# openzklib/openzl

Measured on AMD Instinct MI355X. Metric: MSM points/sec (BLS12-381 G1), higher is better.
Workload: dtype u32; 1 GPU; bls12_381_g1_msm_2^24_per_gpu; points_per_gpu=16777216, curve=BLS12-381 G1, scalars=uniform < r (255 bit), window_bits=20, windows=13, precomputed_table=none (the fixed-key table mode is reported separately as msm_fixed_key), parallelism=single

## Files before the change

### openzl_amd/csrc/zl_msm_accumulate.h

```cpp
#pragma once
#include <type_traits>
#include "zl_ctx.h"
#include "zl_quad.h"
#include "zl_fq2pair.h"
#include "zl_msm_common.h"

__device__ __forceinline__ uint32_t zl_upper_bound(const uint32_t* __restrict__ a, uint32_t n, uint32_t key) {
    uint32_t lo = 0, hi = n;
    while (lo < hi) {
        uint32_t mid = (lo + hi) >> 1;
        if (a[mid] <= key) lo = mid + 1; else hi = mid;
    }
    return lo;
}

#ifndef ZL_ACC_WAVES
#define ZL_ACC_WAVES 2
#endif
#ifndef ZL_ACC_BLOCK
#define ZL_ACC_BLOCK 64
#endif
template <class G, bool QUAD = false>
__device__ __forceinline__ void zl_accumulate_chunk(uint32_t t, int sub, uint32_t E, const uint32_t* __restrict__ entries, const uint32_t* __restrict__ offsets, uint32_t NB,
                                                    const Affine<typename HotField<typename G::F>::type>* __restrict__ bases,
                                                    XYZZ<typename HotField<typename G::F>::type>* __restrict__ bucket_sums,
                                                    XYZZ<typename HotField<typename G::F>::type>* __restrict__ partials, uint32_t ZL_CHUNK,
                                                    const Affine<typename HotField<typename G::F>::type>* __restrict__ phib, uint32_t n_real, uint32_t idx_mask = 0x7fffffffu) {
    using F = typename HotField<typename G::F>::type;
    const uint64_t start64 = (uint64_t)t * ZL_CHUNK;
    if (start64 >= E) return;
    const uint32_t start = (uint32_t)start64;
    const uint32_t end = (uint32_t)min((uint64_t)E, start64 + ZL_CHUNK);
    uint32_t b = zl_upper_bound(offsets, NB + 1, start) - 1;
    uint32_t b_start = offsets[b], b_end = offsets[b + 1];
    XYZZ<F> acc = XYZZ<F>::inf();
    for (uint32_t e = start; e < end; e++) {
        while (e == b_end) {
            if (b_end > b_start) {
                if (!QUAD || sub == 0) {
                    if (b_start >= start) bucket_sums[b] = acc;
                    else partials[(size_t)2 * t] = acc;
                }
                acc = XYZZ<F>::inf();
            }
            b++;
            b_start = b_end;
            b_end = offsets[b + 1];
        }
        const uint32_t ent = entries[e];
        const uint32_t idx = ent & idx_mask;
        const Affine<F> P = (G::GLV && idx >= n_real ? phib : bases)[idx];
        if (!P.is_inf()) {
            if constexpr (QUAD) zl::add_mixed_quad(acc, P.x, P.y, (ent >> 31) != 0, sub);
            else zl::add_mixed(acc, P.x, P.y, (ent >> 31) != 0);
        }
    }
    const bool complete = (b_start >= start) && (b_end <= end);
    if (QUAD && sub != 0) return;
    if (complete) bucket_sums[b] = acc;
    else partials[(size_t)2 * t + (b_start <= start ? 0 : 1)] = acc;
}
template <class G>
__global__ void __launch_bounds__(ZL_ACC_BLOCK, ZL_ACC_WAVES * 64 / ZL_ACC_BLOCK > 0 ? ZL_ACC_WAVES * 64 / ZL_ACC_BLOCK : 1) k_msm_accumulate(const uint32_t* __restrict__ entries, const uint32_t* __restrict__ offsets, uint32_t NB,
                                                        const Affine<typename G::F>* __restrict__ bases_,
                                                        XYZZ<typename G::F>* __restrict__ bucket_sums_,
                                                        XYZZ<typename G::F>* __restrict__ partials_, uint32_t ZL_CHUNK,
                                                        const Affine<typename G::F>* __restrict__ phib_, uint32_t n_real) {
    using F = typename HotField<typename G::F>::type;
    static_assert(sizeof(F) == sizeof(typename G::F), "hot flavour must share the layout");
    zl_accumulate_chunk<G>(blockIdx.x * blockDim.x + threadIdx.x, 0, offsets[NB], entries, offsets, NB, reinterpret_cast<const Affine<F>*>(bases_),
                           reinterpret_cast<XYZZ<F>*>(bucket_sums_), reinterpret_cast<XYZZ<F>*>(partials_), ZL_CHUNK,
                           reinterpret_cast<const Affine<F>*>(phib_) - n_real, n_real);
}
#ifdef ZL_MEASURE
template <class G>
__global__ void __launch_bounds__(ZL_ACC_BLOCK, ZL_ACC_WAVES * 64 / ZL_ACC_BLOCK > 0 ? ZL_ACC_WAVES * 64 / ZL_ACC_BLOCK : 1) k_msm_accumulate_clk(const uint32_t* __restrict__ entries, const uint32_t* __restrict__ offsets, uint32_t NB,
                                                        const Affine<typename G::F>* __restrict__ bases_,
                                                        XYZZ<typename G::F>* __restrict__ bucket_sums_,
                                                        XYZZ<typename G::F>* __restrict__ partials_, uint32_t ZL_CHUNK,
                                                        const Affine<typename G::F>* __restrict__ phib_, uint32_t n_real, unsigned long long* __restrict__ clk, uint32_t idx_mask) {
    if constexpr (G::COORDS == 1) {
        using F = typename HotField<typename G::F>::type;
        const unsigned long long c0 = __builtin_readcyclecounter(), w0 = __builtin_amdgcn_s_memrealtime();
        zl_accumulate_chunk<G>(blockIdx.x * blockDim.x + threadIdx.x, 0, offsets[NB], entries, offsets, NB, reinterpret_cast<const Affine<F>*>(bases_),
                               reinterpret_cast<XYZZ<F>*>(bucket_sums_), reinterpret_cast<XYZZ<F>*>(partials_), ZL_CHUNK,
                               reinterpret_cast<const Affine<F>*>(phib_) - n_real, n_real, idx_mask);
        const unsigned long long c1 = __builtin_readcyclecounter(), w1 = __builtin_amdgcn_s_memrealtime();
        if (threadIdx.x == 0) {
            unsigned long long* o = clk + (size_t)4 * blockIdx.x;
            o[0] = c0; o[1] = c1; o[2] = w0; o[3] = w1;
        }
    }
}
#endif
template <class G>
__global__ void __launch_bounds__(ZL_ACC_BLOCK, ZL_ACC_WAVES * 64 / ZL_ACC_BLOCK > 0 ? ZL_ACC_WAVES * 64 / ZL_ACC_BLOCK : 1) k_msm_accumulate_quad(const uint32_t* __restrict__ entries, const uint32_t* __restrict__ offsets, uint32_t NB,
                                                        const Affine<typename G::F>* __restrict__ bases_,
                                                        XYZZ<typename G::F>* __restrict__ bucket_sums_,
                                                        XYZZ<typename G::F>* __restrict__ partials_, uint32_t ZL_CHUNK,
                                                        const Affine<typename G::F>* __restrict__ phib_, uint32_t n_real) {
    using F = typename HotField<typename G::F>::type;
    const uint32_t gt = blockIdx.x * blockDim.x + threadIdx.x;
    zl_accumulate_chunk<G, true>(gt >> 2, (int)(gt & 3u), offsets[NB], entries, offsets, NB, reinterpret_cast<const Affine<F>*>(bases_),
                                 reinterpret_cast<XYZZ<F>*>(bucket_sums_), reinterpret_cast<XYZZ<F>*>(partials_), ZL_CHUNK,
                                 reinterpret_cast<const Affine<F>*>(phib_) - n_real, n_real);
}
#ifndef ZL_ACC_PAIR_WAVES
#define ZL_ACC_PAIR_WAVES 2
#endif
template <class G, bool QUAD = false>
__global__ void __launch_bounds__(64, ZL_ACC_PAIR_WAVES) k_msm_accumulate_pair(const uint32_t* __restrict__ entries, const uint32_t* __restrict__ offsets, uint32_t NB,
                                                        const Affine<typename G::F>* __restrict__ bases_,
                                                        XYZZ<typename G::F>* __restrict__ bucket_sums,
                                                        XYZZ<typename G::F>* __restrict__ partials, uint32_t ZL_CHUNK,
                                                        const Affine<typename G::F>* __restrict__ phib_, uint32_t n_real) {
    using B = typename PairBase<typename G::F>::type;
    static_assert(!std::is_void<B>::value, "lane-pair kernels: Fq2 groups on 28-bit limbs only");
    using H = Fp2H<B>;
    const int half = zl::pair_half(), sub = (int)(threadIdx.x & 3u);
    const uint32_t t = QUAD ? ZL_OCTET_ITEM() : ZL_PAIR_ITEM();
    const uint32_t E = offsets[NB];
    const Affine<typename G::F>* __restrict__ phib = phib_ - n_real;
    const uint64_t start64 = (uint64_t)t * ZL_CHUNK;
    if (start64 >= E) return;
    const uint32_t start = (uint32_t)start64;
    const uint32_t end = (uint32_t)min((uint64_t)E, start64 + ZL_CHUNK);
    uint32_t b = zl_upper_bound(offsets, NB + 1, start) - 1;
    uint32_t b_start = offsets[b], b_end = offsets[b + 1];
    XYZZ<H> acc = XYZZ<H>::inf();
    for (uint32_t e = start; e < end; e++) {
        while (e == b_end) {
            if (b_end > b_start) {
                if (b_start >= start) pair_store(&bucket_sums[b], half, acc);
                else pair_store(&partials[(size_t)2 * t], half, acc);
                acc = XYZZ<H>::inf();
            }
            b++;
            b_start = b_end;
            b_end = offsets[b + 1];
        }
        const uint32_t ent = entries[e];
        const uint32_t idx = ent & 0x7fffffffu;
        const Affine<H> P = pair_load(&(G::GLV && idx >= n_real ? phib : bases_)[idx], half);
        if (!P.is_inf()) {
            if constexpr (QUAD) zl::add_mixed_quad(acc, P.x, P.y, (ent >> 31) != 0, sub);
            else zl::add_mixed(acc, P.x, P.y, (ent >> 31) != 0);
        }
    }
    const bool complete = (b_start >= start) && (b_end <= end);
    if (complete) pair_store(&bucket_sums[b], half, acc);
    else pair_store(&partials[(size_t)2 * t + (b_start <= start ? 0 : 1)], half, acc);
}
#ifdef ZL_MEASURE
#define ZL_MSM_ACCUMULATE_CLK_KERNEL(X, G) X template __global__ void k_msm_accumulate_clk<G>(const uint32_t*, const uint32_t*, uint32_t, const Affine<typename G::F>*, XYZZ<typename G::F>*, XYZZ<typename G::F>*, uint32_t, const Affine<typename G::F>*, uint32_t, unsigned long long*, uint32_t);
#else
#define ZL_MSM_ACCUMULATE_CLK_KERNEL(X, G)
#endif
#define ZL_MSM_ACCUMULATE_KERNELS_G1(X, G) \
    ZL_MSM_ACCUMULATE_CLK_KERNEL(X, G) \
    X template __global__ void k_msm_accumulate<G>(const uint32_t*, const uint32_t*, uint32_t, const Affine<typename G::F>*, XYZZ<typename G::F>*, XYZZ<typename G::F>*, uint32_t, const Affine<typename G::F>*, uint32_t); \
    X template __global__ void k_msm_accumulate_quad<G>(const uint32_t*, const uint32_t*, uint32_t, const Affine<typename G::F>*, XYZZ<typename G::F>*, XYZZ<typename G::F>*, uint32_t, const Affine<typename G::F>*, uint32_t);
#define ZL_MSM_ACCUMULATE_KERNELS_G2(X, G) \
    X template __global__ void k_msm_accumulate_pair<G, true>(const uint32_t*, const uint32_t*, uint32_t, const Affine<typename G::F>*, XYZZ<typename G::F>*, XYZZ<typename G::F>*, uint32_t, const Affine<typename G::F>*, uint32_t); \
    X template __global__ void k_msm_accumulate_pair<G, false>(const uint32_t*, const uint32_t*, uint32_t, const Affine<typename G::F>*, XYZZ<typename G::F>*, XYZZ<typename G::F>*, uint32_t, const Affine<typename G::F>*, uint32_t);
```

### openzl_amd/csrc/zl_msm_job.h

```cpp
#pragma once
#include <chrono>
#include <stdlib.h>
#include <string.h>
#include <stdio.h>
#include <algorithm>
#include <vector>
#include "zl_ctx.h"
#include "zl_pool.h"
#include "zl_msm_sort.h"
#include "zl_msm_endo.h"
#include "zl_msm_accumulate.h"
#include "zl_msm_reduce.h"

#ifndef ZL_GLS_HOLE_LO_LOG
#define ZL_GLS_HOLE_LO_LOG 11
#define ZL_GLS_HOLE_HI_LOG 17
#define ZL_GLS_END_LOG 19
#endif
static_assert(ZL_GLS_HOLE_LO_LOG >= 0 && ZL_GLS_HOLE_LO_LOG <= ZL_GLS_HOLE_HI_LOG && ZL_GLS_HOLE_HI_LOG <= ZL_GLS_END_LOG && ZL_GLS_END_LOG <= 32, "split below 2^END outside [2^LO, 2^HI)");

static int zl_pick_window(size_t n, int sc_bits, bool wide16 = false ) {
    const double per_bucket = (double)zl_tune("ZL_TUNE_BUCKET_COST_X10", sc_bits > 200 ? 45 : 52) / 10.0;
    double best = 1e300;
    int best_c = 2;
    for (int c = 2; c <= 20; c++) {
        int W = (sc_bits + 1 + c - 1) / c;
        if (c > 16 && (((uint64_t)W << (c - 1)) >> 15) > 255) continue;
        const bool lds_sort = c < 16 || (c == 16 && !wide16);
        double cost = (double)n * W * (lds_sort ? 1.10 : 1.0) + per_bucket * W * (double)(1u << (c - 1));
        if (cost < best) { best = cost; best_c = c; }
    }
    return best_c;
}

static int zl_pick_window_half(size_t n_points) {
    if (n_points < 2) return 0;
    int lg = 63 - __builtin_clzll((unsigned long long)n_points);
    if ((double)n_points >= 1.4142 * (double)((size_t)1 << lg)) lg++;
    static const signed char best[9] = {9, 0, 11, 12, 0, 0, 0, 16, 0};
    return lg >= 11 && lg <= 19 ? best[lg - 11] : 0;
}
static int zl_pick_window_quarter(size_t n_points) {
    if (n_points < 2) return 0;
    int lg = 63 - __builtin_clzll((unsigned long long)n_points);
    if ((double)n_points >= 1.4142 * (double)((size_t)1 << lg)) lg++;
    static const signed char best[9] = {9, 0, 11, 12, 13, 13, 13, 13, 14};
    return lg >= 10 && lg <= 18 ? best[lg - 10] : 0;
}

static int zl_pick_window_precomp(size_t n, int sc_bits) {
    if (n < (size_t)700000) return 16;
    if (n < ((size_t)1 << 21)) return 20;
    double best = 1e300;
    int best_c = 16;
    for (int c = 20; c <= 23; c++) {
        int W = (sc_bits + 1 + c - 1) / c;
        double cost = (double)n * W + 6.0 * (double)(1u << (c - 1));
        if (cost < best) { best = cost; best_c = c; }
    }
    return best_c;
}

struct MsmSortLayout {
    size_t a_bytes = 0, b_bytes = 0;
    uint32_t nslices = 0, per_slice = 0;
    size_t hi8 = 0, part_lo = 0, part_idx = 0, pcounts = 0, idx2 = 0, counts2 = 0;
    uint32_t P = 0, pscan_blocks = 0, fsl = 0, P2 = 0, p2scan_blocks = 0;
    size_t slice_counts = 0;
    size_t vs = 0;
};
template <class G>
struct MsmJob {
    using F = typename G::F;
    using X = XYZZ<F>;
    bool pre = false;
    int c = 0, W = 0;
    int spread_t = -1;
    bool wide = false;
    bool glv = false;
    bool phi_cached = false;
    bool phi_owner = false;
    int sc_bits = 0, endo_k = 1;
    zl_slot phi_slot = ZL_SLOT_PHI_ONE_KEY;
    MsmSortLayout lay;
    unsigned char *d_sort_a = nullptr, *d_sort_b = nullptr;
    size_t n_real = 0;
    uint32_t* d_vs = nullptr;
    const Affine<F>* d_phi = nullptr;
    uint32_t H = 0, SETS = 0, NB = 0, ZL_CHUNK = 0, nchunks = 0, scan_blocks = 0, max_big = 0, max_giant = 0, Gn = 0, big_span = ZL_BIG_SPAN;
    uint32_t red_g0 = 0, red_lg0 = 0, red_blocks = 0, red_levels = 0;
    uint32_t roots_per_set = 0;
    uint64_t maxE = 0;
    size_t n = 0, first = 0;
    const zl_bases* bsp = nullptr;
    uint32_t *d_counts = nullptr, *d_offsets = nullptr, *d_cursor = nullptr, *d_entries = nullptr, *d_block_sums = nullptr, *d_big_list = nullptr,
             *d_big_count = nullptr, *d_ones_count = nullptr, *d_giant_count = nullptr, *d_giant_list = nullptr, *d_ones_list = nullptr,
             *d_bigsg_items = nullptr, *d_bad_scalar = nullptr;
    unsigned long long* d_bigsg_head = nullptr;
    X *d_buckets = nullptr, *d_partials = nullptr, *d_segs = nullptr, *d_stage1 = nullptr, *d_sets = nullptr, *d_ones_parts = nullptr, *d_giant_tmp = nullptr;
    const Affine<F>* d_bases = nullptr;
    const uint8_t* d_inf = nullptr;
    const uint32_t* sc = nullptr;
    X* hw = nullptr;
    uint32_t* hE = nullptr;
    std::vector<X> hw_own;
    void set_host_buffer(X* buf) {
        hw = buf;
        hE = reinterpret_cast<uint32_t*>(buf + (size_t)SETS * roots_per_set + 1);
    }

    int plan(zl_ctx* ctx, const zl_bases& bs, size_t first_, const void* d_scalars, size_t n_, zl_slot phi_slot_) {
        static const bool no_glv = getenv("ZL_NO_GLV") != nullptr;
        bool try_glv = false;
        static const size_t glv_max = (size_t)1 << zl_tune("ZL_TUNE_GLV_MAX_LOG", 19);
        if constexpr (G::GLV) try_glv = bs.precomp_c == 0 && !no_glv && n_ >= 1 && n_ <= glv_max && (uint64_t)n_ * G::ENDO_K < (1ull << 31);
        if constexpr (G::GLV && G::ENDO_K == 2) {
            if constexpr (G::GLVP::LATTICE) {
                if (n_ >= ((size_t)1 << 13) && n_ < ((size_t)1 << 17)) try_glv = false;
            }
        }
        if constexpr (G::GLV && G::ENDO_K == 4) {
            if constexpr (G::GLVP::LATTICE) {
                if (((uint64_t)n_ >= (1ull << ZL_GLS_HOLE_LO_LOG) && (uint64_t)n_ < (1ull << ZL_GLS_HOLE_HI_LOG)) || (uint64_t)n_ >= (1ull << ZL_GLS_END_LOG)) try_glv = false;
            }
        }
        int rc = plan_as(ctx, bs, first_, d_scalars, n_, try_glv);
        if (!rc && glv && c <= 3) rc = plan_as(ctx, bs, first_, d_scalars, n_, false);
        if (!rc && glv && !wide && c > 16) rc = plan_as(ctx, bs, first_, d_scalars, n_, false);
        phi_slot = phi_slot_;
        phi_owner = glv;
        return rc;
    }
    int plan_as(zl_ctx* ctx, const zl_bases& bs, size_t first_, const void* d_scalars, size_t n_, bool glv_) {
        glv = glv_;
        n_real = n_;
        endo_k = glv ? (int)G::ENDO_K : 1;
        n = (size_t)endo_k * n_;
        sc_bits = !glv ? (int)G::SC_BITS : MsmJobPartBits<G>::value;
        first = first_;
        bsp = &bs;
        pre = bs.precomp_c > 0;
        c = pre ? bs.precomp_c : (ctx->msm_c > 0 ? ctx->msm_c : zl_pick_window(n, sc_bits, glv && G::ENDO_K != 2));
        if (!pre && ctx->msm_c <= 0 && glv) {
            int h = 0;
            if constexpr (G::ENDO_K == 2) {
                if (!G::GLVP::LATTICE) h = zl_pick_window_half(n_);
            } else {
                h = zl_pick_window_quarter(n_);
            }
            if (h) c = h;
        }
        if (c < 2) c = 2;
        if (c > 24) c = 24;
        W = (sc_bits + 1 + c - 1) / c;
        H = 1u << (c - 1);
        SETS = pre ? 1u : (uint32_t)W;
        const uint64_t NB64 = (uint64_t)SETS * H;
        maxE = (uint64_t)n * W;
        if (n >= (1ull << 31) || maxE >= (1ull << 32) || NB64 >= (1ull << 31)) return ZL_EINVAL;
        if (pre && (uint64_t)W * bs.n >= (1ull << 31)) return ZL_EINVAL;
        NB = (uint32_t)NB64;
        Gn = NB >> 15;
        if (pre && (c < 16 || Gn < 1 || Gn > 255)) return ZL_EINVAL;
        wide = pre || ((c > 16 || (glv && c == 16 && G::ENDO_K != 2)) && Gn >= 1 && Gn <= 255);
        ZL_CHUNK = (maxE >> 7) >= (1u << 20) ? 128u : (uint32_t)ZL_CHUNK_MAX;
        while (ZL_CHUNK > 8 && maxE / ZL_CHUNK < (1u << 18)) ZL_CHUNK >>= 1;
        uint32_t dense = glv && G::ENDO_K == 2 ? 2u : 1u;
        if constexpr (G::GLV && G::ENDO_K == 4) {
            if constexpr (G::GLVP::LATTICE) {
                static_assert(G::GLVP::PEAK_PCT <= 400, "the top window's busiest buckets are more than 4x the average: a factor of 2 no longer keeps them below 8 chunks");
                if (glv && G::GLVP::PEAK_PCT > 200) dense = 2u;
            }
        }
        while (ZL_CHUNK < (uint32_t)ZL_CHUNK_MAX && dense * (maxE / std::max<uint64_t>(1, (uint64_t)SETS * H)) > (uint64_t)4 * ZL_CHUNK) ZL_CHUNK <<= 1;
        ZL_CHUNK = (uint32_t)std::max(8, zl_tune("ZL_TUNE_CHUNK", (int)ZL_CHUNK));
        nchunks = (uint32_t)((maxE + ZL_CHUNK - 1) / ZL_CHUNK);
        {
            uint32_t g0 = NB >= (1u << 20) ? 8u : (NB >= (1u << 17) ? 4u : 2u);
            g0 = (uint32_t)std::max(2, zl_tune("ZL_TUNE_SEG", (int)g0));
            while (g0 & (g0 - 1)) g0 &= g0 - 1;
            if (g0 > H) g0 = H;
            spread_t = -1;
            if ((wide || c <= 16) && !pre) {
                const int top_bits = sc_bits + 1 - (W - 1) * c;
                if (top_bits - 1 < c - 1) {
                    spread_t = top_bits - 1;
                    if (spread_t > 0 && (1u << spread_t) < g0) g0 = 1u << spread_t;
                }
            }
            red_g0 = g0;
            red_lg0 = 31 - __builtin_clz(g0);
            red_blocks = H / g0;
            red_levels = 31 - __builtin_clz(red_blocks);
            roots_per_set = red_levels + 2;
        }
        scan_blocks = (NB + SCAN_BLOCK * SCAN_ITEMS - 1) / (SCAN_BLOCK * SCAN_ITEMS);
        big_span = nchunks <= (1u << 17) ? (uint32_t)ZL_BIG_SPAN_SMALL : (uint32_t)ZL_BIG_SPAN;
        max_big = (uint32_t)(maxE / ((uint64_t)ZL_CHUNK * big_span)) + 1;
        max_giant = (uint32_t)(maxE / ((uint64_t)ZL_CHUNK * ZL_GIANT_SPAN)) + 1;
        lay = MsmSortLayout{};
        auto up256 = [](size_t b) { return (b + 255) / 256 * 256; };
        const uint32_t max_slices = (uint32_t)((n + 4095) / 4096);
        if (wide) {
            lay.nslices = std::min<uint32_t>(64, max_slices);
            lay.P = Gn * W * lay.nslices;
            lay.pscan_blocks = (lay.P + SCAN_BLOCK * SCAN_ITEMS - 1) / (SCAN_BLOCK * SCAN_ITEMS);
            const size_t b_lo = up256((size_t)n * W * 2), b_hi = up256((size_t)n * W), b_idx = up256((size_t)n * W * 4);
            lay.hi8 = b_lo;
            lay.part_lo = lay.hi8 + b_hi;
            lay.part_idx = lay.part_lo + b_lo;
            lay.pcounts = lay.part_idx + b_idx;
            lay.a_bytes = lay.pcounts + up256((size_t)(2 * lay.P + lay.pscan_blocks + 8) * 4) + 256;
            lay.fsl = 16;
            while (lay.fsl * Gn < 2048 && lay.fsl < 128) lay.fsl *= 2;
            lay.P2 = Gn * 128 * lay.fsl;
            lay.p2scan_blocks = (lay.P2 + SCAN_BLOCK * SCAN_ITEMS - 1) / (SCAN_BLOCK * SCAN_ITEMS);
            lay.idx2 = b_lo;
            lay.counts2 = lay.idx2 + b_idx;
            lay.b_bytes = lay.counts2 + up256((size_t)(2 * (size_t)lay.P2 + lay.p2scan_blocks + 8) * 4) + 256;
        } else if (c <= 16) {
            lay.nslices = std::max<uint32_t>(1, std::min<uint32_t>((256 + W - 1) / W, max_slices));
            lay.slice_counts = up256((size_t)n * W * 2);
            lay.a_bytes = (size_t)n * W * 2 + (size_t)lay.nslices * NB * 4 + 256;
        }
        if (lay.nslices) lay.per_slice = (uint32_t)((n + lay.nslices - 1) / lay.nslices);
        if (glv) {
            lay.vs = up256(lay.a_bytes);
            lay.a_bytes = lay.vs + up256((size_t)n * 32);
        }
        d_bases = pre ? reinterpret_cast<const Affine<F>*>(bs.d_table) : reinterpret_cast<const Affine<F>*>(bs.d_pts) + first;
        d_inf = bs.d_inf ? reinterpret_cast<const uint8_t*>(bs.d_inf) + first : nullptr;
        sc = reinterpret_cast<const uint32_t*>(d_scalars);
        hw_own.assign((size_t)SETS * roots_per_set + 2, X::inf());
        set_host_buffer(hw_own.data());
        return ZL_OK;
    }
    int alloc(zl_ctx* ctx, int set, bool own_sort = false) {
        void* p;
        int rc;
        const zl_msm_set_slots& slots = ZL_MSM_SET[set];
        d_sort_a = d_sort_b = nullptr;
        if (lay.a_bytes) {
            if ((rc = zl_scratch_get(ctx, own_sort ? slots.sort_a : ZL_SLOT_SORT_A, lay.a_bytes, &p))) return rc;
            d_sort_a = (unsigned char*)p;
        }
        if (lay.b_bytes) {
            if ((rc = zl_scratch_get(ctx, own_sort ? slots.sort_b : ZL_SLOT_SORT_B, lay.b_bytes, &p))) return rc;
            d_sort_b = (unsigned char*)p;
        }
        const size_t max_bigsg = (size_t)(maxE / 1024) + 2;
        size_t small_words = (size_t)3 * (NB + 1) + 1 + scan_blocks + 1 + max_big + max_giant + 16 + n + 2 * max_bigsg;
        if ((rc = zl_scratch_get(ctx, slots.data[0], small_words * 4, &p))) return rc;
        d_counts = (uint32_t*)p;
        d_offsets = d_counts + (NB + 1);
        d_cursor = d_offsets + (NB + 2);
        d_block_sums = d_cursor + (NB + 1);
        d_big_list = d_block_sums + scan_blocks + 1;
        d_big_count = d_big_list + max_big;
        d_ones_count = d_big_count + 1;
        d_giant_count = d_big_count + 2;
        d_bad_scalar = d_big_count + 3;
        d_giant_list = d_big_count + 16;
        d_ones_list = d_giant_list + max_giant;
        d_bigsg_items = d_ones_list + n;
        d_bigsg_head = reinterpret_cast<unsigned long long*>((reinterpret_cast<uintptr_t>(d_big_count + 4) + 7) & ~(uintptr_t)7);
        if ((rc = zl_scratch_get(ctx, slots.data[1], maxE * 4, &p))) return rc;
        d_entries = (uint32_t*)p;
        if ((rc = zl_scratch_get(ctx, slots.data[2], (size_t)NB * sizeof(X), &p))) return rc;
        d_buckets = (X*)p;
        if ((rc = zl_scratch_get(ctx, slots.data[3], (size_t)2 * nchunks * sizeof(X), &p))) return rc;
        d_partials = (X*)p;
        const size_t leaf_elems = (size_t)2 * SETS * red_blocks, lvl1_elems = (size_t)3 * SETS * (red_blocks / 2 + 1);
        const size_t root_elems = (size_t)SETS * roots_per_set;
        if ((rc = zl_scratch_get(ctx, slots.tail, (leaf_elems + lvl1_elems + root_elems + 2 + ZL_ONES_BLOCKS + (size_t)max_giant * ZL_GIANT_PARTS) * sizeof(X), &p))) return rc;
        d_segs = (X*)p;
        d_stage1 = d_segs + leaf_elems;
        d_sets = d_stage1 + lvl1_elems;
        d_ones_parts = d_sets + root_elems + 2;
        d_giant_tmp = d_ones_parts + ZL_ONES_BLOCKS;
        if (glv) {
            const size_t endo_bytes = (size_t)(endo_k - 1) * n_real * sizeof(Affine<F>);
            const zl_bases& bs = *bsp;
            std::lock_guard<std::mutex> cache_lk(zl_bases_cache_mutex());
            if (!bs.d_endo && endo_bytes <= ((size_t)zl_tune("ZL_TUNE_ENDO_CACHE_MB", 512) << 20)) {
                void* q = nullptr;
                if (hipMalloc(&q, endo_bytes) == hipSuccess) {
                    if constexpr (G::GLV && G::ENDO_K == 2)
                        hipLaunchKernelGGL((k_glv_phi<G>), dim3((uint32_t)((n_real + 127) / 128)), dim3(128), 0, ctx->stream, d_bases, (uint32_t)n_real, reinterpret_cast<Affine<F>*>(q));
                    else if constexpr (G::GLV && G::ENDO_K == 4)
                        hipLaunchKernelGGL((k_gls_psi<G>), dim3((uint32_t)((n_real + 63) / 64)), dim3(64), 0, ctx->stream, d_bases, (uint32_t)n_real, reinterpret_cast<Affine<F>*>(q));
                    if (hipGetLastError() != hipSuccess || hipStreamSynchronize(ctx->stream) != hipSuccess) { (void)hipFree(q); return ZL_EHIP; }
                    bs.d_endo = q;
                    bs.endo_first = first;
                    bs.endo_n = n_real;
                    bs.endo_k = endo_k;
                } else {
                    (void)hipGetLastError();
                }
            }
            if (bs.d_endo && bs.endo_first == first && bs.endo_n == n_real && bs.endo_k == endo_k) {
                d_phi = reinterpret_cast<const Affine<F>*>(bs.d_endo);
                phi_owner = false;
                phi_cached = true;
            }
        }
        if (glv && phi_owner) {
            if ((rc = zl_scratch_get(ctx, phi_slot, (size_t)(endo_k - 1) * n_real * sizeof(Affine<F>), &p))) return rc;
            d_phi = reinterpret_cast<const Affine<F>*>(p);
        }
        return ZL_OK;
    }
    int sort(zl_ctx* ctx, hipStream_t st) {
        if (!wide && c > 16) ZL_HIP(ctx, hipMemsetAsync(d_counts, 0, (size_t)(NB + 1) * 4, st));
        hipLaunchKernelGGL(k_msm_zero_words, dim3(1), dim3(64), 0, st, d_big_count, 8u);
        const uint32_t nblk = (uint32_t)((n + 255) / 256);
        const uint32_t* sc_eff = sc;
        const uint8_t* inf_eff = d_inf;
        uint32_t* bad_eff = d_bad_scalar;
        if (glv) {
            d_vs = reinterpret_cast<uint32_t*>(d_sort_a + lay.vs);
            if constexpr (G::GLV && G::ENDO_K == 2) {
                if constexpr (G::GLVP::LATTICE)
                    hipLaunchKernelGGL((k_glv_split_lattice<typename G::GLVP>), dim3((uint32_t)((n_real + 255) / 256)), dim3(256), 0, st, sc, (uint32_t)n_real, d_inf, d_vs, (int)G::SC_BITS, d_bad_scalar);
                else
                    hipLaunchKernelGGL((k_glv_split<typename G::GLVP>), dim3((uint32_t)((n_real + 255) / 256)), dim3(256), 0, st, sc, (uint32_t)n_real, d_inf, d_vs, (int)G::SC_BITS, d_bad_scalar);
                if (phi_owner)
                    hipLaunchKernelGGL((k_glv_phi<G>), dim3((uint32_t)((n_real + 127) / 128)), dim3(128), 0, st, d_bases, (uint32_t)n_real, const_cast<Affine<F>*>(d_phi));
            } else if constexpr (G::GLV && G::ENDO_K == 4) {
                if constexpr (G::GLVP::LATTICE)
                    hipLaunchKernelGGL((k_gls_split_lattice<typename G::GLVP>), dim3((uint32_t)((n_real + 255) / 256)), dim3(256), 0, st, sc, (uint32_t)n_real, d_inf, d_vs, (int)G::SC_BITS, d_bad_scalar);
                else
                    hipLaunchKernelGGL((k_gls_split<typename G::GLVP>), dim3((uint32_t)((n_real + 255) / 256)), dim3(256), 0, st, sc, (uint32_t)n_real, d_inf, d_vs, (int)G::SC_BITS, d_bad_scalar);
                if (phi_owner)
                    hipLaunchKernelGGL((k_gls_psi<G>), dim3((uint32_t)((n_real + 63) / 64)), dim3(64), 0, st, d_bases, (uint32_t)n_real, const_cast<Affine<F>*>(d_phi));
            }
            sc_eff = d_vs;
            inf_eff = nullptr;
            bad_eff = nullptr;
        }
        const int glv_i = glv ? 1 : 0;
        (void)hipFuncSetAttribute(reinterpret_cast<const void*>(&k_msm_hist_lds), hipFuncAttributeMaxDynamicSharedMemorySize, 128 * 1024);
        (void)hipFuncSetAttribute(reinterpret_cast<const void*>(&k_msm_scatter_range), hipFuncAttributeMaxDynamicSharedMemorySize, 128 * 1024);
        if (wide) sort_wide(st, sc_eff, inf_eff, bad_eff, nblk, glv_i);
        else if (c <= 16) sort_lds(st, sc_eff, inf_eff, bad_eff, nblk, glv_i);
        else sort_atomics(st, nblk);
        ZL_HIP(ctx, hipGetLastError());
        return ZL_OK;
    }
    void sort_wide(hipStream_t st, const uint32_t* sc_eff, const uint8_t* inf_eff, uint32_t* bad_eff, uint32_t nblk, int glv_i) {
        const zl_bases& bs = *bsp;
        const uint32_t nslices = lay.nslices, per_slice = lay.per_slice, P = lay.P, pscan_blocks = lay.pscan_blocks;
        uint16_t* d_lo16 = (uint16_t*)d_sort_a;
        uint8_t* d_hi8 = (uint8_t*)(d_sort_a + lay.hi8);
        uint16_t* d_part_lo = (uint16_t*)(d_sort_a + lay.part_lo);
        uint32_t* d_part_idx = (uint32_t*)(d_sort_a + lay.part_idx);
        uint32_t* d_pcounts = (uint32_t*)(d_sort_a + lay.pcounts);
        uint32_t* d_poff = d_pcounts + P;
        uint32_t* d_pblock = d_poff + P + 1;
        hipLaunchKernelGGL(k_msm_recode_wide, dim3(nblk), dim3(256), 0, st, sc_eff, (uint32_t)n, c, W, pre ? 0u : (H >> 15), spread_t, glv_i, d_lo16, d_hi8, d_ones_list, d_ones_count, inf_eff, sc_bits, bad_eff);
        hipLaunchKernelGGL(k_msm_part_hist, dim3(nslices, W), dim3(256), 0, st, d_hi8, (uint32_t)n, (uint32_t)W, Gn, per_slice, nslices, d_pcounts);
        hipLaunchKernelGGL(k_scan_block_sums, dim3(pscan_blocks), dim3(SCAN_BLOCK), 0, st, d_pcounts, P, d_pblock);
        hipLaunchKernelGGL(k_scan_top, dim3(1), dim3(1024), 0, st, d_pblock, pscan_blocks, d_poff + P, (const uint32_t*)nullptr);
        hipLaunchKernelGGL(k_scan_apply, dim3(pscan_blocks), dim3(SCAN_BLOCK), 0, st, d_pcounts, P, d_pblock, d_poff, d_pcounts);
        hipLaunchKernelGGL(k_msm_part_scatter_st, dim3(nslices, W), dim3(256), 0, st, d_lo16, d_hi8, (uint32_t)n, (uint32_t)W, Gn, per_slice, nslices, d_poff,
                           pre ? (uint32_t)bs.n : 0u, pre ? (uint32_t)first : 0u, d_part_lo, d_part_idx);
        const uint32_t gstride = (uint32_t)W * nslices;
        const uint32_t SG = Gn * 128;
        const uint32_t fsl = lay.fsl, P2 = lay.P2, p2scan_blocks = lay.p2scan_blocks;
        uint16_t* d_lo2 = (uint16_t*)d_sort_b;
        uint32_t* d_idx2 = (uint32_t*)(d_sort_b + lay.idx2);
        uint32_t* d_c2 = (uint32_t*)(d_sort_b + lay.counts2);
        uint32_t* d_off2 = d_c2 + P2;
        uint32_t* d_blk2 = d_off2 + P2 + 1;
        hipLaunchKernelGGL(k_msm_sub_hist, dim3(fsl, Gn), dim3(256), 0, st, d_part_lo, d_poff, Gn, gstride, d_poff + P, fsl, d_c2);
        hipLaunchKernelGGL(k_scan_block_sums, dim3(p2scan_blocks), dim3(SCAN_BLOCK), 0, st, d_c2, P2, d_blk2);
        hipLaunchKernelGGL(k_scan_top, dim3(1), dim3(1024), 0, st, d_blk2, p2scan_blocks, d_off2 + P2, (const uint32_t*)nullptr);
        hipLaunchKernelGGL(k_scan_apply, dim3(p2scan_blocks), dim3(SCAN_BLOCK), 0, st, d_c2, P2, d_blk2, d_off2, d_c2);
        hipLaunchKernelGGL(k_msm_sub_scatter_st, dim3(fsl, Gn), dim3(256), 0, st, d_part_lo, d_part_idx, d_poff, Gn, gstride, d_poff + P, fsl, d_off2, d_lo2,
                           d_idx2);
        hipLaunchKernelGGL(k_msm_fine_hist, dim3(SG), dim3(256), 0, st, d_lo2, d_off2, SG, fsl, d_off2 + P2, d_counts);
        hipLaunchKernelGGL(k_scan_block_sums, dim3(scan_blocks), dim3(SCAN_BLOCK), 0, st, d_counts, NB, d_block_sums);
        hipLaunchKernelGGL(k_scan_top, dim3(1), dim3(1024), 0, st, d_block_sums, scan_blocks, d_offsets + NB, (const uint32_t*)d_bad_scalar);
        hipLaunchKernelGGL(k_scan_apply, dim3(scan_blocks), dim3(SCAN_BLOCK), 0, st, d_counts, NB, d_block_sums, d_offsets, d_cursor);
        uint32_t cap = (uint32_t)std::min<uint64_t>(36 * 1024, std::max<uint64_t>(4096, (maxE / SG) * 22 / 10));
        cap = (uint32_t)std::max(1024, zl_tune("ZL_TUNE_FS_CAP", (int)cap));
        (void)hipFuncSetAttribute(reinterpret_cast<const void*>(&k_msm_fine_sort), hipFuncAttributeMaxDynamicSharedMemorySize, 160 * 1024);
        hipLaunchKernelGGL(k_msm_fine_sort, dim3(SG), dim3(zl_tune("ZL_TUNE_FS", 1024)), (size_t)(256 + cap) * 4, st, d_lo2, d_idx2, d_off2, SG, fsl, d_off2 + P2, d_offsets, cap,
                           d_entries, d_bigsg_head, d_bigsg_items);
        (void)hipFuncSetAttribute(reinterpret_cast<const void*>(&k_msm_fine_sort_big), hipFuncAttributeMaxDynamicSharedMemorySize, ZL_BT * 4);
        hipLaunchKernelGGL(k_msm_fine_sort_big, dim3(512), dim3(1024), (size_t)ZL_BT * 4, st, d_lo2, d_idx2, d_off2, SG, fsl, d_off2 + P2, d_bigsg_head,
                           d_bigsg_items, d_cursor, d_entries);
    }
    void sort_lds(hipStream_t st, const uint32_t* sc_eff, const uint8_t* inf_eff, uint32_t* bad_eff, uint32_t nblk, int glv_i) {
        const uint32_t nslices = lay.nslices, per_slice = lay.per_slice;
        uint16_t* d_digits = (uint16_t*)d_sort_a;
        uint32_t* d_slice_counts = (uint32_t*)(d_sort_a + lay.slice_counts);
        hipLaunchKernelGGL(k_msm_recode, dim3(nblk), dim3(256), 0, st, sc_eff, (uint32_t)n, c, W, spread_t, glv_i, d_digits, d_ones_list, d_ones_count, inf_eff, sc_bits, bad_eff);
        hipLaunchKernelGGL(k_msm_hist_lds, dim3(nslices, W), dim3(1024), (size_t)H * 4, st, d_digits, (uint32_t)n, H, per_slice, NB, d_slice_counts);
        if (NB <= 14336 && nslices <= 64) {
            hipLaunchKernelGGL(k_msm_prefix_small, dim3(1), dim3(1024), ((size_t)NB + NB / 16 + 16) * 4, st, d_slice_counts, NB, nslices, d_offsets, d_cursor, (const uint32_t*)d_bad_scalar);
        } else {
        hipLaunchKernelGGL(k_msm_slice_prefix, dim3((NB + 255) / 256), dim3(256), 0, st, d_slice_counts, NB, nslices, d_counts);
        hipLaunchKernelGGL(k_scan_block_sums, dim3(scan_blocks), dim3(SCAN_BLOCK), 0, st, d_counts, NB, d_block_sums);
        hipLaunchKernelGGL(k_scan_top, dim3(1), dim3(1024), 0, st, d_block_sums, scan_blocks, d_offsets + NB, (const uint32_t*)d_bad_scalar);
        hipLaunchKernelGGL(k_scan_apply, dim3(scan_blocks), dim3(SCAN_BLOCK), 0, st, d_counts, NB, d_block_sums, d_offsets, d_cursor);
        }
        uint32_t ranges = 1;
        while (ranges * W < 256 && (H / (ranges * 2)) >= 64) ranges *= 2;
        ranges = (uint32_t)std::max(1, zl_tune("ZL_TUNE_RANGES", (int)ranges));
        const uint32_t RB = (H + ranges - 1) / ranges;
        const uint32_t parts = 1;
        hipLaunchKernelGGL(k_msm_scatter_range, dim3(8 * ((W + 7) / 8), ranges, parts), dim3(1024), (size_t)RB * 4, st, d_digits, (uint32_t)n, H, RB, d_offsets, d_entries,
                           (const uint32_t*)d_slice_counts, NB, nslices, per_slice, parts, (uint32_t)W);
    }
    void sort_atomics(hipStream_t st, uint32_t nblk) {
        hipLaunchKernelGGL((k_msm_digits<0>), dim3(nblk), dim3(256), 0, st, sc, (uint32_t)n, c, W, d_counts, (uint32_t*)nullptr, d_ones_list, d_ones_count, d_inf, (int)G::SC_BITS, d_bad_scalar);
        hipLaunchKernelGGL(k_scan_block_sums, dim3(scan_blocks), dim3(SCAN_BLOCK), 0, st, d_counts, NB, d_block_sums);
        hipLaunchKernelGGL(k_scan_top, dim3(1), dim3(1024), 0, st, d_block_sums, scan_blocks, d_offsets + NB, (const uint32_t*)d_bad_scalar);
        hipLaunchKernelGGL(k_scan_apply, dim3(scan_blocks), dim3(SCAN_BLOCK), 0, st, d_counts, NB, d_block_sums, d_offsets, d_cursor);
        hipLaunchKernelGGL((k_msm_digits<1>), dim3(nblk), dim3(256), 0, st, sc, (uint32_t)n, c, W, d_cursor, d_entries, d_ones_list, d_ones_count, d_inf, (int)G::SC_BITS, d_bad_scalar);
    }
    static constexpr bool pair_ok() { return G::COORDS == 2 && !std::is_void<typename PairBase<F>::type>::value; }
    int accumulate(zl_ctx* ctx, hipStream_t st) {
        static_assert(G::COORDS == 1 || pair_ok(), "every Fq2 group runs on 28-bit limbs: its MSM kernels are the lane-pair ones");
        const bool quad = nchunks <= (uint64_t)zl_tune("ZL_TUNE_QUAD_ACC_CHUNKS", 24576);
        if constexpr (pair_ok()) {
            if (quad)
                hipLaunchKernelGGL((k_msm_accumulate_pair<G, true>), dim3((nchunks + 7) / 8), dim3(64), 0, st, d_entries, d_offsets, NB, d_bases, d_buckets, d_partials, ZL_CHUNK,
                                   glv ? d_phi : d_bases, glv ? (uint32_t)n_real : 0xFFFFFFFFu);
            else
                hipLaunchKernelGGL((k_msm_accumulate_pair<G, false>), dim3((nchunks + 31) / 32), dim3(64), 0, st, d_entries, d_offsets, NB, d_bases, d_buckets, d_partials, ZL_CHUNK,
                                   glv ? d_phi : d_bases, glv ? (uint32_t)n_real : 0xFFFFFFFFu);
        } else {
            if (quad)
                hipLaunchKernelGGL((k_msm_accumulate_quad<G>), dim3((4 * nchunks + ZL_ACC_BLOCK - 1) / ZL_ACC_BLOCK), dim3(ZL_ACC_BLOCK), 0, st, d_entries, d_offsets, NB, d_bases, d_buckets, d_partials, ZL_CHUNK,
                                   glv ? d_phi : d_bases, glv ? (uint32_t)n_real : 0xFFFFFFFFu);
#ifdef ZL_MEASURE
            else if (ctx->acc_clk && (size_t)((nchunks + ZL_ACC_BLOCK - 1) / ZL_ACC_BLOCK) * 32 <= ctx->acc_clk_cap) {
                ctx->acc_clk_waves = (nchunks + ZL_ACC_BLOCK - 1) / ZL_ACC_BLOCK;
                hipLaunchKernelGGL((k_msm_accumulate_clk<G>), dim3((nchunks + ZL_ACC_BLOCK - 1) / ZL_ACC_BLOCK), dim3(ZL_ACC_BLOCK), 0, st, d_entries, d_offsets, NB, d_bases, d_buckets, d_partials, ZL_CHUNK,
                                   glv ? d_phi : d_bases, glv ? (uint32_t)n_real : 0xFFFFFFFFu, (unsigned long long*)ctx->acc_clk,
                                   zl_tune("ZL_TUNE_ACC_CLK_IDX_BITS", 31) >= 31 ? 0x7fffffffu : ((1u << zl_tune("ZL_TUNE_ACC_CLK_IDX_BITS", 31)) - 1u));
            }
#endif
            else
                hipLaunchKernelGGL((k_msm_accumulate<G>), dim3((nchunks + ZL_ACC_BLOCK - 1) / ZL_ACC_BLOCK), dim3(ZL_ACC_BLOCK), 0, st, d_entries, d_offsets, NB, d_bases, d_buckets, d_partials, ZL_CHUNK,
                                   glv ? d_phi : d_bases, glv ? (uint32_t)n_real : 0xFFFFFFFFu);
        }
        ZL_HIP(ctx, hipGetLastError());
        return ZL_OK;
    }
    int tail(zl_ctx* ctx, hipStream_t st) {
        const uint32_t quad_max = (uint32_t)zl_tune("ZL_TUNE_QUAD_LANES", 65536);
        const bool by_cuts = NB > quad_max && nchunks > 1;
        if (by_cuts) hipLaunchKernelGGL((k_msm_fill_empty<G>), dim3((NB + 255) / 256), dim3(256), 0, st, d_offsets, NB, d_buckets);
        if constexpr (pair_ok()) {
            if (by_cuts)
                hipLaunchKernelGGL((k_msm_merge_cuts_pair<G>), dim3((nchunks + 31) / 32), dim3(64), 0, st, d_offsets, NB, d_buckets, d_partials, d_big_list, d_big_count, d_giant_list, d_giant_count, ZL_CHUNK, big_span, nchunks);
            else if (NB > quad_max)
                hipLaunchKernelGGL((k_msm_merge_pair<G, false>), dim3((NB + 31) / 32), dim3(64), 0, st, d_offsets, NB, d_buckets, d_partials, d_big_list, d_big_count, d_giant_list, d_giant_count, ZL_CHUNK, big_span);
            else
                hipLaunchKernelGGL((k_msm_merge_pair<G, true>), dim3((NB + 7) / 8), dim3(64), 0, st, d_offsets, NB, d_buckets, d_partials, d_big_list, d_big_count, d_giant_list, d_giant_count, ZL_CHUNK, big_span);
        } else {
            if (by_cuts)
                hipLaunchKernelGGL((k_msm_merge_cuts<G>), dim3((nchunks + 63) / 64), dim3(64), 0, st, d_offsets, NB, d_buckets, d_partials, d_big_list, d_big_count, d_giant_list, d_giant_count, ZL_CHUNK, big_span, nchunks);
            else if (NB > quad_max)
                hipLaunchKernelGGL((k_msm_merge<G>), dim3((NB + 63) / 64), dim3(64), 0, st, d_offsets, NB, d_buckets, d_partials, d_big_list, d_big_count, d_giant_list, d_giant_count, ZL_CHUNK, big_span);
            else
                hipLaunchKernelGGL((k_msm_merge<G, true>), dim3((4 * NB + 63) / 64), dim3(64), 0, st, d_offsets, NB, d_buckets, d_partials, d_big_list, d_big_count, d_giant_list, d_giant_count, ZL_CHUNK, big_span);
        }
        const bool may_big = nchunks > big_span, may_giant = nchunks > (uint32_t)ZL_GIANT_SPAN;
        if constexpr (pair_ok()) {
            if (may_big) hipLaunchKernelGGL((k_msm_merge_big_pair<G>), dim3(std::min<uint32_t>(max_big, 1024)), dim3(2 * TreeLanes<G>::N), TreeLanes<G>::N * sizeof(X), st, d_offsets, d_buckets,
                               d_partials, d_big_list, d_big_count, ZL_CHUNK);
            if (may_giant) hipLaunchKernelGGL((k_msm_merge_giant_pair<G>), dim3(std::min<uint32_t>(max_giant, 16) * ZL_GIANT_PARTS), dim3(2 * TreeLanes<G>::N), TreeLanes<G>::N * sizeof(X), st,
                               d_offsets, d_giant_tmp, d_partials, d_giant_list, d_giant_count, ZL_CHUNK);
            if (may_giant) hipLaunchKernelGGL((k_msm_merge_giant2_pair<G>), dim3(std::min<uint32_t>(max_giant, 64)), dim3(2 * ZL_GIANT_PARTS), 0, st, d_buckets, d_giant_tmp, d_giant_list, d_giant_count);
        } else {
            if (may_big) hipLaunchKernelGGL((k_msm_merge_big<G>), dim3(std::min<uint32_t>(max_big, 1024)), dim3(TreeLanes<G>::N), TreeLanes<G>::N * sizeof(X), st, d_offsets, d_buckets,
                           d_partials, d_big_list, d_big_count, ZL_CHUNK);
            if (may_giant) hipLaunchKernelGGL((k_msm_merge_giant<G>), dim3(std::min<uint32_t>(max_giant, 16) * ZL_GIANT_PARTS), dim3(TreeLanes<G>::N), TreeLanes<G>::N * sizeof(X), st,
                           d_offsets, d_giant_tmp, d_partials, d_giant_list, d_giant_count, ZL_CHUNK);
            if (may_giant) hipLaunchKernelGGL((k_msm_merge_giant2<G>), dim3((max_giant + 63) / 64), dim3(64), 0, st, d_buckets, d_giant_tmp, d_giant_list, d_giant_count);
        }
        hipLaunchKernelGGL((k_msm_ones<G>), dim3(ZL_ONES_BLOCKS), dim3(TreeLanes<G>::N), TreeLanes<G>::N * sizeof(X), st, d_ones_list, d_ones_count,
                           pre ? d_bases + first : d_bases, d_ones_parts, glv ? d_phi : d_bases, glv ? (uint32_t)n_real : 0xFFFFFFFFu,
                           d_sets + (size_t)SETS * roots_per_set, d_big_count + 6, (const uint32_t*)(d_offsets + NB));
        {
            const uint32_t fset = spread_t >= 0 ? (uint32_t)(W - 1) : 0xFFFFFFFFu, flog = (uint32_t)std::max(spread_t, 0);
            const uint32_t leaves = SETS * red_blocks;
            X* cur = red_levels == 0 ? d_sets : d_segs;
            if constexpr (pair_ok()) {
                if (leaves > quad_max)
                    hipLaunchKernelGGL((k_msm_reduce_level0_pair<G, false>), dim3((leaves + 31) / 32), dim3(64), 0, st, d_buckets, H, red_g0, red_blocks, leaves, fset, flog, cur);
                else
                    hipLaunchKernelGGL((k_msm_reduce_level0_pair<G, true>), dim3((leaves + 7) / 8), dim3(64), 0, st, d_buckets, H, red_g0, red_blocks, leaves, fset, flog, cur);
            } else {
                if (leaves > quad_max)
                    hipLaunchKernelGGL((k_msm_reduce_level0<G>), dim3((leaves + 63) / 64), dim3(64), 0, st, d_buckets, H, red_g0, red_blocks, leaves, fset, flog, cur);
                else
                    hipLaunchKernelGGL((k_msm_reduce_level0<G, true>), dim3((4 * leaves + 63) / 64), dim3(64), 0, st, d_buckets, H, red_g0, red_blocks, leaves, fset, flog, cur);
            }
            for (uint32_t lv = 1; lv <= red_levels; lv++) {
                const uint32_t nodes = red_blocks >> lv, lanes = SETS * nodes * (lv + 2);
                X* nxt = lv == red_levels ? d_sets : ((lv & 1) ? d_stage1 : d_segs);
                if constexpr (pair_ok()) {
                    if (lanes > quad_max)
                        hipLaunchKernelGGL((k_msm_reduce_tree_pair<G, false>), dim3((lanes + 31) / 32), dim3(64), 0, st, cur, nxt, lv, nodes, lanes);
                    else
                        hipLaunchKernelGGL((k_msm_reduce_tree_pair<G, true>), dim3((lanes + 7) / 8), dim3(64), 0, st, cur, nxt, lv, nodes, lanes);
                } else {
                    if (lanes > quad_max)
                        hipLaunchKernelGGL((k_msm_reduce_tree<G>), dim3((lanes + 63) / 64), dim3(64), 0, st, cur, nxt, lv, nodes, lanes);
                    else
                        hipLaunchKernelGGL((k_msm_reduce_tree<G, true>), dim3((4 * lanes + 63) / 64), dim3(64), 0, st, cur, nxt, lv, nodes, lanes);
                }
                cur = nxt;
            }
        }
        ZL_HIP(ctx, hipGetLastError());
        ZL_HIP(ctx, hipMemcpyAsync(hw, d_sets, sizeof(X) * ((size_t)SETS * roots_per_set + 1) + 8, hipMemcpyDeviceToHost, st));
        return ZL_OK;
    }
    X window_value(int w) const {
        const X* root = hw + (size_t)w * roots_per_set;
        X v = X::inf();
        const int top = (int)red_lg0 + (int)red_levels - 1;
        for (int off = std::max(top, 0); off >= 0; off--) {
            if (off != std::max(top, 0)) zl::dbl_inplace(v);
            const int bsel = off - (int)red_lg0;
            if (bsel >= 0 && bsel < (int)red_levels) {
                const bool skipped = spread_t >= 0 && w == (int)SETS - 1 && off >= spread_t && !pre;
                if (!skipped) zl::add_full(v, root[2 + bsel]);
            }
            if (off == 0) zl::add_full(v, root[1]);
        }
        return v;
    }
    X finish(bool parallel = true, double* values_us = nullptr) const {
        std::vector<X> V(SETS);
        const auto t0 = std::chrono::steady_clock::now();
        if (parallel && SETS >= 4) zl_pool_get().parallel_for(SETS, [&](size_t w) { V[w] = window_value((int)w); });
        else for (uint32_t w = 0; w < SETS; w++) V[w] = window_value((int)w);
        if (values_us) *values_us = (double)std::chrono::duration_cast<std::chrono::nanoseconds>(std::chrono::steady_clock::now() - t0).count() / 1e3;
        X total = V[SETS - 1];
        for (int w = (int)SETS - 2; w >= 0; w--) {
            zl::dbl_n(total, c);
            zl::add_full(total, V[w]);
        }
        zl::add_full(total, hw[(size_t)SETS * roots_per_set]);
        return total;
    }
};
```

### openzl_amd/csrc/zl_msm_reduce.h

```cpp
#pragma once
#include "zl_ctx.h"
#include <type_traits>
#include "zl_quad.h"
#include "zl_fq2pair.h"
#include "zl_msm_common.h"

template <class G, bool QUAD = false>
__global__ void __launch_bounds__(64, (QUAD && sizeof(XYZZ<typename G::F>) <= 256) ? 3 : 1) k_msm_merge(const uint32_t* __restrict__ offsets, uint32_t NB, XYZZ<typename G::F>* __restrict__ bucket_sums,
                                                   const XYZZ<typename G::F>* __restrict__ partials, uint32_t* __restrict__ big_list,
                                                   uint32_t* __restrict__ big_count, uint32_t* __restrict__ giant_list, uint32_t* __restrict__ giant_count,
                                                   uint32_t ZL_CHUNK, uint32_t big_span) {
    ZL_SIDE_PRIO();
    using F = typename G::F;
    const uint32_t gt = blockIdx.x * blockDim.x + threadIdx.x;
    const uint32_t b = QUAD ? gt >> 2 : gt;
    const int sub = QUAD ? (int)(gt & 3u) : 0;
    if (b >= NB) return;
    const uint32_t s = offsets[b], e = offsets[b + 1];
    if (s == e) { if (sub == 0) bucket_sums[b] = XYZZ<F>::inf(); return; }
    const uint32_t t0 = s / ZL_CHUNK, t1 = (e - 1) / ZL_CHUNK;
    if (t0 == t1) return;
    if (t1 - t0 + 1 > ZL_GIANT_SPAN) { if (sub == 0) giant_list[atomicAdd(giant_count, 1u)] = b; return; }
    if (t1 - t0 + 1 > big_span) { if (sub == 0) big_list[atomicAdd(big_count, 1u)] = b; return; }
    XYZZ<F> acc = XYZZ<F>::inf();
    for (uint32_t t = t0; t <= t1; t++) {
        const XYZZ<F> p = partials[(size_t)2 * t + (s <= t * ZL_CHUNK ? 0 : 1)];
        if constexpr (QUAD) zl::add_full_quad(acc, p, sub);
        else zl::add_full(acc, p);
    }
    if (sub == 0) bucket_sums[b] = acc;
}
__device__ __forceinline__ uint32_t zl_bucket_of_entry(const uint32_t* __restrict__ offsets, uint32_t NB, uint32_t p) {
    uint32_t lo = 0, hi = NB + 1;
    while (lo < hi) {
        const uint32_t mid = (lo + hi) >> 1;
        if (offsets[mid] <= p) lo = mid + 1; else hi = mid;
    }
    return lo - 1;
}
template <class G>
__global__ void __launch_bounds__(256) k_msm_fill_empty(const uint32_t* __restrict__ offsets, uint32_t NB, XYZZ<typename G::F>* __restrict__ bucket_sums) {
    ZL_SIDE_PRIO();
    const uint32_t b = blockIdx.x * blockDim.x + threadIdx.x;
    if (b >= NB || offsets[b] != offsets[b + 1]) return;
    bucket_sums[b] = XYZZ<typename G::F>::inf();
}
template <class G>
__global__ void __launch_bounds__(64, sizeof(XYZZ<typename G::F>) <= 256 ? 3 : 1) k_msm_merge_cuts(const uint32_t* __restrict__ offsets, uint32_t NB, XYZZ<typename G::F>* __restrict__ bucket_sums,
                                                   const XYZZ<typename G::F>* __restrict__ partials, uint32_t* __restrict__ big_list,
                                                   uint32_t* __restrict__ big_count, uint32_t* __restrict__ giant_list, uint32_t* __restrict__ giant_count,
                                                   uint32_t ZL_CHUNK, uint32_t big_span, uint32_t nchunks) {
    ZL_SIDE_PRIO();
    using F = typename G::F;
    const uint32_t t = blockIdx.x * blockDim.x + threadIdx.x + 1;
    if (t >= nchunks) return;
    const uint64_t p64 = (uint64_t)t * ZL_CHUNK;
    if (p64 >= offsets[NB]) return;
    const uint32_t p = (uint32_t)p64;
    const uint32_t b = zl_bucket_of_entry(offsets, NB, p);
    const uint32_t s = offsets[b], e = offsets[b + 1];
    if (s == p || s / ZL_CHUNK != t - 1) return;
    const uint32_t t0 = t - 1, t1 = (e - 1) / ZL_CHUNK;
    if (t1 - t0 + 1 > ZL_GIANT_SPAN) { giant_list[atomicAdd(giant_count, 1u)] = b; return; }
    if (t1 - t0 + 1 > big_span) { big_list[atomicAdd(big_count, 1u)] = b; return; }
    XYZZ<F> acc = XYZZ<F>::inf();
    for (uint32_t tt = t0; tt <= t1; tt++) {
        const XYZZ<F> q = partials[(size_t)2 * tt + (s <= tt * ZL_CHUNK ? 0 : 1)];
        zl::add_full(acc, q);
    }
    bucket_sums[b] = acc;
}
template <class G>
struct TreeLanes { static constexpr int N = sizeof(XYZZ<typename G::F>) > 256 ? 128 : 256; };
template <class G>
__device__ __forceinline__ void zl_block_tree(XYZZ<typename G::F>* sh, XYZZ<typename G::F>& acc) {
    using F = typename G::F;
    sh[threadIdx.x] = acc;
    __syncthreads();
    for (int off = TreeLanes<G>::N / 2; off > 0; off >>= 1) {
        if ((int)threadIdx.x < off) {
            XYZZ<F> a = sh[threadIdx.x];
            const XYZZ<F> o = sh[threadIdx.x + off];
            zl::add_full(a, o);
            sh[threadIdx.x] = a;
        }
        __syncthreads();
    }
    acc = sh[0];
    __syncthreads();
}
template <class G>
__global__ void __launch_bounds__(TreeLanes<G>::N) k_msm_merge_big(const uint32_t* __restrict__ offsets, XYZZ<typename G::F>* __restrict__ bucket_sums,
                                                        const XYZZ<typename G::F>* __restrict__ partials, const uint32_t* __restrict__ big_list,
                                                        const uint32_t* __restrict__ big_count, uint32_t ZL_CHUNK) {
    ZL_SIDE_PRIO();
    using F = typename G::F;
    extern __shared__ __attribute__((aligned(16))) unsigned char smem[];
    XYZZ<F>* sh = reinterpret_cast<XYZZ<F>*>(smem);
    for (uint32_t item = blockIdx.x; item < *big_count; item += gridDim.x) {
        const uint32_t b = big_list[item];
        const uint32_t s = offsets[b], e = offsets[b + 1];
        const uint32_t t0 = s / ZL_CHUNK, t1 = (e - 1) / ZL_CHUNK;
        XYZZ<F> acc = XYZZ<F>::inf();
        for (uint32_t t = t0 + threadIdx.x; t <= t1; t += blockDim.x) {
            const XYZZ<F> p = partials[(size_t)2 * t + (s <= t * ZL_CHUNK ? 0 : 1)];
            zl::add_full(acc, p);
        }
        zl_block_tree<G>(sh, acc);
        if (threadIdx.x == 0) bucket_sums[b] = acc;
    }
}
template <class G>
__global__ void __launch_bounds__(TreeLanes<G>::N) k_msm_merge_giant(const uint32_t* __restrict__ offsets, XYZZ<typename G::F>* __restrict__ giant_tmp,
                                                          const XYZZ<typename G::F>* __restrict__ partials, const uint32_t* __restrict__ giant_list,
                                                          const uint32_t* __restrict__ giant_count, uint32_t ZL_CHUNK) {
    ZL_SIDE_PRIO();
    using F = typename G::F;
    extern __shared__ __attribute__((aligned(16))) unsigned char smem[];
    XYZZ<F>* sh = reinterpret_cast<XYZZ<F>*>(smem);
    const uint32_t part = blockIdx.x % ZL_GIANT_PARTS;
    for (uint32_t item = blockIdx.x / ZL_GIANT_PARTS; item < *giant_count; item += gridDim.x / ZL_GIANT_PARTS) {
        const uint32_t b = giant_list[item];
        const uint32_t s = offsets[b], e = offsets[b + 1];
        const uint32_t t0 = s / ZL_CHUNK, t1 = (e - 1) / ZL_CHUNK;
        const uint32_t per = (t1 - t0 + ZL_GIANT_PARTS) / ZL_GIANT_PARTS;
        const uint32_t lo = t0 + part * per, hi = min(t1 + 1, lo + per);
        XYZZ<F> acc = XYZZ<F>::inf();
        for (uint32_t t = lo + threadIdx.x; t < hi; t += blockDim.x) {
            const XYZZ<F> p = partials[(size_t)2 * t + (s <= t * ZL_CHUNK ? 0 : 1)];
            zl::add_full(acc, p);
        }
        zl_block_tree<G>(sh, acc);
        if (threadIdx.x == 0) giant_tmp[(size_t)item * ZL_GIANT_PARTS + part] = acc;
    }
}
template <class G>
__global__ void __launch_bounds__(64) k_msm_merge_giant2(XYZZ<typename G::F>* __restrict__ bucket_sums, const XYZZ<typename G::F>* __restrict__ giant_tmp,
                                                          const uint32_t* __restrict__ giant_list, const uint32_t* __restrict__ giant_count) {
    ZL_SIDE_PRIO();
    using F = typename G::F;
    const uint32_t item = blockIdx.x * blockDim.x + threadIdx.x;
    if (item >= *giant_count) return;
    XYZZ<F> acc = XYZZ<F>::inf();
    for (uint32_t k = 0; k < ZL_GIANT_PARTS; k++) {
        const XYZZ<F> p = giant_tmp[(size_t)item * ZL_GIANT_PARTS + k];
        zl::add_full(acc, p);
    }
    bucket_sums[giant_list[item]] = acc;
}
#define ZL_ONES_BLOCKS 128

template <class X>
__device__ __forceinline__ X zl_load_volatile(const X* p) {
    X r;
    const volatile uint32_t* s = reinterpret_cast<const volatile uint32_t*>(p);
    uint32_t* d = reinterpret_cast<uint32_t*>(&r);
#pragma unroll
    for (int i = 0; i < (int)(sizeof(X) / 4); i++) d[i] = s[i];
    return r;
}
template <class G>
__global__ void __launch_bounds__(TreeLanes<G>::N) k_msm_ones(const uint32_t* __restrict__ ones_list, const uint32_t* __restrict__ ones_count,
                                                   const Affine<typename G::F>* __restrict__ bases, XYZZ<typename G::F>* __restrict__ out,
                                                   const Affine<typename G::F>* __restrict__ phib, uint32_t n_real, XYZZ<typename G::F>* __restrict__ final_out,
                                                   uint32_t* __restrict__ done, const uint32_t* __restrict__ status_in) {
    ZL_SIDE_PRIO();
    using F = typename G::F;
    extern __shared__ __attribute__((aligned(16))) unsigned char smem[];
    XYZZ<F>* sh = reinterpret_cast<XYZZ<F>*>(smem);
    __shared__ uint32_t last_flag;
    const uint32_t cnt = *ones_count;
    if (blockIdx.x == 0 && threadIdx.x == 0) {
        uint32_t* st = reinterpret_cast<uint32_t*>(final_out + 1);
        st[0] = status_in[0];
        st[1] = status_in[1];
    }
    if (cnt == 0) {
        if (blockIdx.x == 0 && threadIdx.x == 0) *final_out = XYZZ<F>::inf();
        return;
    }
    const uint32_t nparts = min(gridDim.x, (cnt + blockDim.x - 1) / blockDim.x);
    if (blockIdx.x >= nparts) return;
    XYZZ<F> acc = XYZZ<F>::inf();
    for (uint32_t j = blockIdx.x * blockDim.x + threadIdx.x; j < cnt; j += nparts * blockDim.x) {
        const uint32_t idx = ones_list[j];
        const Affine<F> P = (G::GLV && idx >= n_real) ? phib[idx - n_real] : bases[idx];
        if (!P.is_inf()) zl::add_mixed(acc, P.x, P.y, false);
    }
    if (cnt > 1) zl_block_tree<G>(sh, acc);
    if (nparts == 1) {
        if (threadIdx.x == 0) *final_out = acc;
        return;
    }
    if (threadIdx.x == 0) {
        out[blockIdx.x] = acc;
        __threadfence();
        last_flag = atomicAdd(done, 1u) == nparts - 1 ? 1u : 0u;
    }
    __syncthreads();
    if (!last_flag) return;
    __threadfence();
    acc = XYZZ<F>::inf();
    for (uint32_t s = threadIdx.x; s < nparts; s += blockDim.x) {
        const XYZZ<F> p = zl_load_volatile(&out[s]);
        zl::add_full(acc, p);
    }
    zl_block_tree<G>(sh, acc);
    if (threadIdx.x == 0) *final_out = acc;
}

template <class G, bool QUAD = false>
__global__ void __launch_bounds__(64, TreeLanes<G>::N == 128 ? 1 : 2) k_msm_reduce_level0(const XYZZ<typename G::F>* __restrict__ buckets, uint32_t H, uint32_t group, uint32_t blocks_per_set,
                                                           uint32_t total_blocks, uint32_t flat_set, uint32_t flat_log,
                                                           XYZZ<typename G::F>* __restrict__ out ) {
    ZL_SIDE_PRIO();
    using X = XYZZ<typename G::F>;
    const uint32_t gt = blockIdx.x * blockDim.x + threadIdx.x;
    const uint32_t t = QUAD ? gt >> 2 : gt;
    const int sub = QUAD ? (int)(gt & 3u) : 0;
    if (t >= total_blocks) return;
    const uint32_t set = t / blocks_per_set, blk = t % blocks_per_set;
    const uint32_t i0 = blk * group, i1 = min(H, i0 + group);
    const size_t base = (size_t)set * H;
    const bool flat = set == flat_set && flat_log == 0;
    X run = X::inf(), wsum = X::inf();
    for (uint32_t i = i1; i > i0; i--) {
        const X B = buckets[base + (i - 1)];
        if constexpr (QUAD) {
            zl::add_full_quad(run, B, sub);
            if (!flat) zl::add_full_quad(wsum, run, sub);
        } else {
            zl::add_full(run, B);
            if (!flat) zl::add_full(wsum, run);
        }
    }
    if (sub != 0) return;
    out[(size_t)2 * t] = run;
    if (flat) out[(size_t)2 * t + 1] = run;
    else out[(size_t)2 * t + 1] = wsum;
}
template <class G, bool QUAD = false>
__global__ void __launch_bounds__(64) k_msm_reduce_tree(const XYZZ<typename G::F>* __restrict__ in, XYZZ<typename G::F>* __restrict__ out, uint32_t level,
                                                         uint32_t nodes_out_per_set, uint32_t total_lanes) {
    ZL_SIDE_PRIO();
    using X = XYZZ<typename G::F>;
    const uint32_t gt = blockIdx.x * blockDim.x + threadIdx.x;
    const uint32_t t = QUAD ? gt >> 2 : gt;
    const int sub = QUAD ? (int)(gt & 3u) : 0;
    if (t >= total_lanes) return;
    const uint32_t ch_out = level + 2, ch_in = level + 1;
    const uint32_t ch = t % ch_out, node = (t / ch_out) % nodes_out_per_set, set = t / (ch_out * nodes_out_per_set);
    const size_t left = ((size_t)set * nodes_out_per_set * 2 + (size_t)2 * node) * ch_in, right = left + ch_in;
    if (ch == ch_out - 1) {
        if (sub == 0) out[t] = in[right];
        return;
    }
    X acc = in[left + ch];
    const X o = in[right + ch];
    if constexpr (QUAD) zl::add_full_quad(acc, o, sub);
    else zl::add_full(acc, o);
    if (sub == 0) out[t] = acc;
}
template <class G, bool QUAD = false>
__global__ void __launch_bounds__(64, 2) k_msm_merge_pair(const uint32_t* __restrict__ offsets, uint32_t NB, XYZZ<typename G::F>* __restrict__ bucket_sums,
                                                   const XYZZ<typename G::F>* __restrict__ partials, uint32_t* __restrict__ big_list,
                                                   uint32_t* __restrict__ big_count, uint32_t* __restrict__ giant_list, uint32_t* __restrict__ giant_count,
                                                   uint32_t ZL_CHUNK, uint32_t big_span) {
    using B = typename PairBase<typename G::F>::type;
    static_assert(!std::is_void<B>::value, "lane-pair kernels: Fq2 groups on 28-bit limbs only");
    ZL_SIDE_PRIO();
    using X = XYZZ<Fp2H<B>>;
    const int half = zl::pair_half(), sub = (int)(threadIdx.x & 3u);
    const uint32_t b = QUAD ? ZL_OCTET_ITEM() : ZL_PAIR_ITEM();
    if (b >= NB) return;
    const uint32_t s = offsets[b], e = offsets[b + 1];
    if (s == e) { pair_store(&bucket_sums[b], half, X::inf()); return; }
    const uint32_t t0 = s / ZL_CHUNK, t1 = (e - 1) / ZL_CHUNK;
    if (t0 == t1) return;
    const bool first = half == 0 && (!QUAD || sub == 0);
    if (t1 - t0 + 1 > ZL_GIANT_SPAN) { if (first) giant_list[atomicAdd(giant_count, 1u)] = b; return; }
    if (t1 - t0 + 1 > big_span) { if (first) big_list[atomicAdd(big_count, 1u)] = b; return; }
    X acc = X::inf();
    for (uint32_t t = t0; t <= t1; t++) {
        const X p = pair_load(&partials[(size_t)2 * t + (s <= t * ZL_CHUNK ? 0 : 1)], half);
        if constexpr (QUAD) zl::add_full_quad(acc, p, sub);
        else zl::add_full(acc, p);
    }
    pair_store(&bucket_sums[b], half, acc);
}
template <class G>
__global__ void __launch_bounds__(64, 2) k_msm_merge_cuts_pair(const uint32_t* __restrict__ offsets, uint32_t NB, XYZZ<typename G::F>* __restrict__ bucket_sums,
                                                   const XYZZ<typename G::F>* __restrict__ partials, uint32_t* __restrict__ big_list,
                                                   uint32_t* __restrict__ big_count, uint32_t* __restrict__ giant_list, uint32_t* __restrict__ giant_count,
                                                   uint32_t ZL_CHUNK, uint32_t big_span, uint32_t nchunks) {
    using B = typename PairBase<typename G::F>::type;
    static_assert(!std::is_void<B>::value, "lane-pair kernels: Fq2 groups on 28-bit limbs only");
    ZL_SIDE_PRIO();
    using X = XYZZ<Fp2H<B>>;
    const int half = zl::pair_half();
    const uint32_t t = ZL_PAIR_ITEM() + 1;
    if (t >= nchunks) return;
    const uint64_t p64 = (uint64_t)t * ZL_CHUNK;
    if (p64 >= offsets[NB]) return;
    const uint32_t p = (uint32_t)p64;
    const uint32_t b = zl_bucket_of_entry(offsets, NB, p);
    const uint32_t s = offsets[b], e = offsets[b + 1];
    if (s == p || s / ZL_CHUNK != t - 1) return;
    const uint32_t t0 = t - 1, t1 = (e - 1) / ZL_CHUNK;
    if (t1 - t0 + 1 > ZL_GIANT_SPAN) { if (half == 0) giant_list[atomicAdd(giant_count, 1u)] = b; return; }
    if (t1 - t0 + 1 > big_span) { if (half == 0) big_list[atomicAdd(big_count, 1u)] = b; return; }
    X acc = X::inf();
    for (uint32_t tt = t0; tt <= t1; tt++) {
        const X q = pair_load(&partials[(size_t)2 * tt + (s <= tt * ZL_CHUNK ? 0 : 1)], half);
        zl::add_full(acc, q);
    }
    pair_store(&bucket_sums[b], half, acc);
}
#ifndef ZL_L0_PAIR_WAVES
#define ZL_L0_PAIR_WAVES 2
#endif
template <class G, bool QUAD = false>
__global__ void __launch_bounds__(64, ZL_L0_PAIR_WAVES) k_msm_reduce_level0_pair(const XYZZ<typename G::F>* __restrict__ buckets, uint32_t H, uint32_t group, uint32_t blocks_per_set,
                                                           uint32_t total_blocks, uint32_t flat_set, uint32_t flat_log, XYZZ<typename G::F>* __restrict__ out) {
    using B = typename PairBase<typename G::F>::type;
    static_assert(!std::is_void<B>::value, "lane-pair kernels: Fq2 groups on 28-bit limbs only");
    ZL_SIDE_PRIO();
    using X = XYZZ<Fp2H<B>>;
    const int half = zl::pair_half(), sub = (int)(threadIdx.x & 3u);
    const uint32_t t = QUAD ? ZL_OCTET_ITEM() : ZL_PAIR_ITEM();
    if (t >= total_blocks) return;
    const uint32_t set = t / blocks_per_set, blk = t % blocks_per_set;
    const uint32_t i0 = blk * group, i1 = min(H, i0 + group);
    const size_t base = (size_t)set * H;
    const bool flat = set == flat_set && flat_log == 0;
    X run = X::inf(), wsum = X::inf();
    for (uint32_t i = i1; i > i0; i--) {
        const X Bk = pair_load(&buckets[base + (i - 1)], half);
        if constexpr (QUAD) {
            zl::add_full_quad(run, Bk, sub);
            if (!flat) zl::add_full_quad(wsum, run, sub);
        } else {
            zl::add_full(run, Bk);
            if (!flat) zl::add_full(wsum, run);
        }
    }
    pair_store(&out[(size_t)2 * t], half, run);
    if (flat) pair_store(&out[(size_t)2 * t + 1], half, run);
    else pair_store(&out[(size_t)2 * t + 1], half, wsum);
}
template <class G, bool QUAD = false>
__global__ void __launch_bounds__(64, 2) k_msm_reduce_tree_pair(const XYZZ<typename G::F>* __restrict__ in, XYZZ<typename G::F>* __restrict__ out, uint32_t level,
                                                         uint32_t nodes_out_per_set, uint32_t total_lanes) {
    using B = typename PairBase<typename G::F>::type;
    static_assert(!std::is_void<B>::value, "lane-pair kernels: Fq2 groups on 28-bit limbs only");
    ZL_SIDE_PRIO();
    using X = XYZZ<Fp2H<B>>;
    const int half = zl::pair_half(), sub = (int)(threadIdx.x & 3u);
    const uint32_t t = QUAD ? ZL_OCTET_ITEM() : ZL_PAIR_ITEM();
    if (t >= total_lanes) return;
    const uint32_t ch_out = level + 2, ch_in = level + 1;
    const uint32_t ch = t % ch_out, node = (t / ch_out) % nodes_out_per_set, set = t / (ch_out * nodes_out_per_set);
    const size_t left = ((size_t)set * nodes_out_per_set * 2 + (size_t)2 * node) * ch_in, right = left + ch_in;
    if (ch == ch_out - 1) {
        pair_store(&out[t], half, pair_load(&in[right], half));
        return;
    }
    X acc = pair_load(&in[left + ch], half);
    const X o = pair_load(&in[right + ch], half);
    if constexpr (QUAD) zl::add_full_quad(acc, o, sub);
    else zl::add_full(acc, o);
    pair_store(&out[t], half, acc);
}
#define ZL_PAIR_ITEM_IN_BLOCK() (((threadIdx.x >> 4) << 3) + (threadIdx.x & 7u))
template <class G, int N>
__device__ __forceinline__ void zl_block_tree_pair(XYZZ<typename G::F>* sh, XYZZ<Fp2H<typename PairBase<typename G::F>::type>>& acc, uint32_t item, int half) {
    using X = XYZZ<Fp2H<typename PairBase<typename G::F>::type>>;
    pair_store(&sh[item], half, acc);
    __syncthreads();
    for (uint32_t off = N / 2; off > 0; off >>= 1) {
        if (item < off) {
            X a = pair_load(&sh[item], half);
            const X o = pair_load(&sh[item + off], half);
            zl::add_full(a, o);
            pair_store(&sh[item], half, a);
        }
        __syncthreads();
    }
    acc = pair_load(&sh[0], half);
    __syncthreads();
}
template <class G>
__global__ void __launch_bounds__(2 * TreeLanes<G>::N) k_msm_merge_big_pair(const uint32_t* __restrict__ offsets, XYZZ<typename G::F>* __restrict__ bucket_sums,
                                                        const XYZZ<typename G::F>* __restrict__ partials, const uint32_t* __restrict__ big_list,
                                                        const uint32_t* __restrict__ big_count, uint32_t ZL_CHUNK) {
    using B = typename PairBase<typename G::F>::type;
    static_assert(!std::is_void<B>::value, "lane-pair kernels: Fq2 groups on 28-bit limbs only");
    ZL_SIDE_PRIO();
    using X = XYZZ<Fp2H<B>>;
    constexpr uint32_t N = TreeLanes<G>::N;
    extern __shared__ __attribute__((aligned(16))) unsigned char smem[];
    XYZZ<typename G::F>* sh = reinterpret_cast<XYZZ<typename G::F>*>(smem);
    const int half = zl::pair_half();
    const uint32_t item = ZL_PAIR_ITEM_IN_BLOCK();
    for (uint32_t it = blockIdx.x; it < *big_count; it += gridDim.x) {
        const uint32_t b = big_list[it];
        const uint32_t s = offsets[b], e = offsets[b + 1];
        const uint32_t t0 = s / ZL_CHUNK, t1 = (e - 1) / ZL_CHUNK;
        X acc = X::inf();
        for (uint32_t t = t0 + item; t <= t1; t += N) {
            const X p = pair_load(&partials[(size_t)2 * t + (s <= t * ZL_CHUNK ? 0 : 1)], half);
            zl::add_full(acc, p);
        }
        zl_block_tree_pair<G, N>(sh, acc, item, half);
        if (item == 0) pair_store(&bucket_sums[b], half, acc);
    }
}
template <class G>
__global__ void __launch_bounds__(2 * TreeLanes<G>::N) k_msm_merge_giant_pair(const uint32_t* __restrict__ offsets, XYZZ<typename G::F>* __restrict__ giant_tmp,
                                                          const XYZZ<typename G::F>* __restrict__ partials, const uint32_t* __restrict__ giant_list,
                                                          const uint32_t* __restrict__ giant_count, uint32_t ZL_CHUNK) {
    using B = typename PairBase<typename G::F>::type;
    static_assert(!std::is_void<B>::value, "lane-pair kernels: Fq2 groups on 28-bit limbs only");
    ZL_SIDE_PRIO();
    using X = XYZZ<Fp2H<B>>;
    constexpr uint32_t N = TreeLanes<G>::N;
    extern __shared__ __attribute__((aligned(16))) unsigned char smem[];
    XYZZ<typename G::F>* sh = reinterpret_cast<XYZZ<typename G::F>*>(smem);
    const int half = zl::pair_half();
    const uint32_t item = ZL_PAIR_ITEM_IN_BLOCK();
    const uint32_t part = blockIdx.x % ZL_GIANT_PARTS;
    for (uint32_t it = blockIdx.x / ZL_GIANT_PARTS; it < *giant_count; it += gridDim.x / ZL_GIANT_PARTS) {
        const uint32_t b = giant_list[it];
        const uint32_t s = offsets[b], e = offsets[b + 1];
        const uint32_t t0 = s / ZL_CHUNK, t1 = (e - 1) / ZL_CHUNK;
        const uint32_t per = (t1 - t0 + ZL_GIANT_PARTS) / ZL_GIANT_PARTS;
        const uint32_t lo = t0 + part * per, hi = min(t1 + 1, lo + per);
        X acc = X::inf();
        for (uint32_t t = lo + item; t < hi; t += N) {
            const X p = pair_load(&partials[(size_t)2 * t + (s <= t * ZL_CHUNK ? 0 : 1)], half);
            zl::add_full(acc, p);
        }
        zl_block_tree_pair<G, N>(sh, acc, item, half);
        if (item == 0) pair_store(&giant_tmp[(size_t)it * ZL_GIANT_PARTS + part], half, acc);
    }
}
template <class G>
__global__ void __launch_bounds__(2 * ZL_GIANT_PARTS) k_msm_merge_giant2_pair(XYZZ<typename G::F>* __restrict__ bucket_sums, XYZZ<typename G::F>* __restrict__ giant_tmp,
                                                          const uint32_t* __restrict__ giant_list, const uint32_t* __restrict__ giant_count) {
    using B = typename PairBase<typename G::F>::type;
    static_assert(!std::is_void<B>::value, "lane-pair kernels: Fq2 groups on 28-bit limbs only");
    ZL_SIDE_PRIO();
    using X = XYZZ<Fp2H<B>>;
    const int half = zl::pair_half();
    const uint32_t item = ZL_PAIR_ITEM_IN_BLOCK();
    for (uint32_t it = blockIdx.x; it < *giant_count; it += gridDim.x) {
        XYZZ<typename G::F>* sh = giant_tmp + (size_t)it * ZL_GIANT_PARTS;
        X acc = pair_load(&sh[item], half);
        __syncthreads();
        zl_block_tree_pair<G, ZL_GIANT_PARTS>(sh, acc, item, half);
        if (item == 0) {
            pair_store(&bucket_sums[giant_list[it]], half, acc);
        }
    }
}

#define ZL_MSM_TAIL_KERNELS_COMMON(X, G) \
    X template __global__ void k_msm_fill_empty<G>(const uint32_t*, uint32_t, XYZZ<typename G::F>*); \
    X template __global__ void k_msm_ones<G>(const uint32_t*, const uint32_t*, const Affine<typename G::F>*, XYZZ<typename G::F>*, const Affine<typename G::F>*, uint32_t, XYZZ<typename G::F>*, uint32_t*, const uint32_t*);
#define ZL_MSM_TAIL_KERNELS_G1(X, G) \
    ZL_MSM_TAIL_KERNELS_COMMON(X, G) \
    X template __global__ void k_msm_merge<G, false>(const uint32_t*, uint32_t, XYZZ<typename G::F>*, const XYZZ<typename G::F>*, uint32_t*, uint32_t*, uint32_t*, uint32_t*, uint32_t, uint32_t); \
    X template __global__ void k_msm_merge<G, true>(const uint32_t*, uint32_t, XYZZ<typename G::F>*, const XYZZ<typename G::F>*, uint32_t*, uint32_t*, uint32_t*, uint32_t*, uint32_t, uint32_t); \
    X template __global__ void k_msm_merge_cuts<G>(const uint32_t*, uint32_t, XYZZ<typename G::F>*, const XYZZ<typename G::F>*, uint32_t*, uint32_t*, uint32_t*, uint32_t*, uint32_t, uint32_t, uint32_t); \
    X template __global__ void k_msm_merge_big<G>(const uint32_t*, XYZZ<typename G::F>*, const XYZZ<typename G::F>*, const uint32_t*, const uint32_t*, uint32_t); \
    X template __global__ void k_msm_merge_giant<G>(const uint32_t*, XYZZ<typename G::F>*, const XYZZ<typename G::F>*, const uint32_t*, const uint32_t*, uint32_t); \
    X template __global__ void k_msm_merge_giant2<G>(XYZZ<typename G::F>*, const XYZZ<typename G::F>*, const uint32_t*, const uint32_t*); \
    X template __global__ void k_msm_reduce_level0<G, false>(const XYZZ<typename G::F>*, uint32_t, uint32_t, uint32_t, uint32_t, uint32_t, uint32_t, XYZZ<typename G::F>*); \
    X template __global__ void k_msm_reduce_level0<G, true>(const XYZZ<typename G::F>*, uint32_t, uint32_t, uint32_t, uint32_t, uint32_t, uint32_t, XYZZ<typename G::F>*); \
    X template __global__ void k_msm_reduce_tree<G, false>(const XYZZ<typename G::F>*, XYZZ<typename G::F>*, uint32_t, uint32_t, uint32_t); \
    X template __global__ void k_msm_reduce_tree<G, true>(const XYZZ<typename G::F>*, XYZZ<typename G::F>*, uint32_t, uint32_t, uint32_t);
#define ZL_MSM_TAIL_KERNELS_G2(X, G) \
    ZL_MSM_TAIL_KERNELS_COMMON(X, G) \
    X template __global__ void k_msm_merge_pair<G, false>(const uint32_t*, uint32_t, XYZZ<typename G::F>*, const XYZZ<typename G::F>*, uint32_t*, uint32_t*, uint32_t*, uint32_t*, uint32_t, uint32_t); \
    X template __global__ void k_msm_merge_pair<G, true>(const uint32_t*, uint32_t, XYZZ<typename G::F>*, const XYZZ<typename G::F>*, uint32_t*, uint32_t*, uint32_t*, uint32_t*, uint32_t, uint32_t); \
    X template __global__ void k_msm_merge_cuts_pair<G>(const uint32_t*, uint32_t, XYZZ<typename G::F>*, const XYZZ<typename G::F>*, uint32_t*, uint32_t*, uint32_t*, uint32_t*, uint32_t, uint32_t, uint32_t); \
    X template __global__ void k_msm_merge_big_pair<G>(const uint32_t*, XYZZ<typename G::F>*, const XYZZ<typename G::F>*, const uint32_t*, const uint32_t*, uint32_t); \
    X template __global__ void k_msm_merge_giant_pair<G>(const uint32_t*, XYZZ<typename G::F>*, const XYZZ<typename G::F>*, const uint32_t*, const uint32_t*, uint32_t); \
    X template __global__ void k_msm_merge_giant2_pair<G>(XYZZ<typename G::F>*, XYZZ<typename G::F>*, const uint32_t*, const uint32_t*); \
    X template __global__ void k_msm_reduce_level0_pair<G, false>(const XYZZ<typename G::F>*, uint32_t, uint32_t, uint32_t, uint32_t, uint32_t, uint32_t, XYZZ<typename G::F>*); \
    X template __global__ void k_msm_reduce_level0_pair<G, true>(const XYZZ<typename G::F>*, uint32_t, uint32_t, uint32_t, uint32_t, uint32_t, uint32_t, XYZZ<typename G::F>*); \
    X template __global__ void k_msm_reduce_tree_pair<G, false>(const XYZZ<typename G::F>*, XYZZ<typename G::F>*, uint32_t, uint32_t, uint32_t); \
    X template __global__ void k_msm_reduce_tree_pair<G, true>(const XYZZ<typename G::F>*, XYZZ<typename G::F>*, uint32_t, uint32_t, uint32_t);
```

### openzl_amd/csrc/zl_msm_sort.h

```cpp
#pragma once
#include "zl_msm_common.h"

#define ZL_PT 4096
#define ZL_BT 16384
#define SCAN_ITEMS 16
#define SCAN_BLOCK 256

__global__ void __launch_bounds__(64) k_msm_zero_words(uint32_t* __restrict__ p, uint32_t n);
template <int MODE>
__global__ void __launch_bounds__(256) k_msm_digits(const uint32_t* __restrict__ scalars, uint32_t n, int c, int W,
                                                    uint32_t* __restrict__ counters, uint32_t* __restrict__ entries,
                                                    uint32_t* __restrict__ ones_list, uint32_t* __restrict__ ones_count, const uint8_t* __restrict__ inf,
                                                    int sc_bits, uint32_t* __restrict__ bad);
__global__ void __launch_bounds__(256) k_msm_recode(const uint32_t* __restrict__ scalars, uint32_t n, int c, int W, int spread_t, int glv, uint16_t* __restrict__ digits,
                                                             uint32_t* __restrict__ ones_list, uint32_t* __restrict__ ones_count, const uint8_t* __restrict__ inf,
                                                             int sc_bits, uint32_t* __restrict__ bad);
__global__ void __launch_bounds__(1024) k_msm_hist_lds(const uint16_t* __restrict__ digits, uint32_t n, uint32_t H, uint32_t per_slice, uint32_t NB,
                                                        uint32_t* __restrict__ counts);
__global__ void __launch_bounds__(256) k_msm_slice_prefix(uint32_t* __restrict__ counts, uint32_t NB, uint32_t nslices, uint32_t* __restrict__ tot);
__global__ void __launch_bounds__(1024) k_msm_scatter_range(const uint16_t* __restrict__ digits, uint32_t n, uint32_t H, uint32_t RB,
                                                                     const uint32_t* __restrict__ offsets, uint32_t* __restrict__ entries,
                                                                     const uint32_t* __restrict__ slice_prefix, uint32_t NB, uint32_t nslices, uint32_t per_slice,
                                                                     uint32_t parts, uint32_t W);
__global__ void __launch_bounds__(256) k_msm_recode_wide(const uint32_t* __restrict__ scalars, uint32_t n, int c, int W, uint32_t gw, int spread_t, int glv,
                                                                  uint16_t* __restrict__ lo16, uint8_t* __restrict__ hi8,
                                                                  uint32_t* __restrict__ ones_list, uint32_t* __restrict__ ones_count, const uint8_t* __restrict__ inf,
                                                                  int sc_bits, uint32_t* __restrict__ bad);
__global__ void __launch_bounds__(256) k_msm_part_hist(const uint8_t* __restrict__ hi8, uint32_t n, uint32_t W, uint32_t G, uint32_t per_slice,
                                                                uint32_t nslices, uint32_t* __restrict__ counts);
__global__ void __launch_bounds__(256) k_msm_sub_hist(const uint16_t* __restrict__ part_lo, const uint32_t* __restrict__ part_off, uint32_t G,
                                                               uint32_t stride, const uint32_t* __restrict__ total, uint32_t fslices,
                                                               uint32_t* __restrict__ counts);
__global__ void __launch_bounds__(256) k_msm_part_scatter_st(const uint16_t* __restrict__ lo16, const uint8_t* __restrict__ hi8, uint32_t n, uint32_t W,
                                                                      uint32_t G, uint32_t per_slice, uint32_t nslices, const uint32_t* __restrict__ part_off,
                                                                      uint32_t table_stride, uint32_t first, uint16_t* __restrict__ out_lo,
                                                                      uint32_t* __restrict__ out_idx);
__global__ void __launch_bounds__(256) k_msm_sub_scatter_st(const uint16_t* __restrict__ part_lo, const uint32_t* __restrict__ part_idx,
                                                                     const uint32_t* __restrict__ part_off, uint32_t G, uint32_t stride,
                                                                     const uint32_t* __restrict__ total, uint32_t fslices, const uint32_t* __restrict__ sub_off,
                                                                     uint16_t* __restrict__ out_lo, uint32_t* __restrict__ out_idx);
__global__ void __launch_bounds__(256) k_msm_fine_hist(const uint16_t* __restrict__ lo2, const uint32_t* __restrict__ sub_off, uint32_t SG,
                                                                uint32_t fslices, const uint32_t* __restrict__ total, uint32_t* __restrict__ counts);
__global__ void __launch_bounds__(1024) k_msm_fine_sort(const uint16_t* __restrict__ lo2, const uint32_t* __restrict__ idx2,
                                                                const uint32_t* __restrict__ sub_off, uint32_t SG, uint32_t fslices,
                                                                const uint32_t* __restrict__ total, const uint32_t* __restrict__ offsets, uint32_t cap,
                                                                uint32_t* __restrict__ entries, unsigned long long* __restrict__ big_head,
                                                                uint32_t* __restrict__ big_items);
__global__ void __launch_bounds__(1024) k_msm_fine_sort_big(const uint16_t* __restrict__ lo2, const uint32_t* __restrict__ idx2,
                                                                    const uint32_t* __restrict__ sub_off, uint32_t SG, uint32_t fslices,
                                                                    const uint32_t* __restrict__ total, const unsigned long long* __restrict__ big_head,
                                                                    const uint32_t* __restrict__ big_items, uint32_t* __restrict__ cursor,
                                                                    uint32_t* __restrict__ entries);
__global__ void __launch_bounds__(SCAN_BLOCK) k_scan_block_sums(const uint32_t* __restrict__ in, uint32_t count, uint32_t* __restrict__ block_sums);
__global__ void __launch_bounds__(1024) k_scan_top(uint32_t* __restrict__ block_sums, uint32_t nblocks, uint32_t* __restrict__ total_out,
                                                          const uint32_t* __restrict__ flag_in = nullptr );
__global__ void __launch_bounds__(1024) k_msm_prefix_small(uint32_t* __restrict__ counts, uint32_t NB, uint32_t nslices, uint32_t* __restrict__ offsets,
                                                                  uint32_t* __restrict__ cursor, const uint32_t* __restrict__ flag_in);
__global__ void __launch_bounds__(SCAN_BLOCK) k_scan_apply(const uint32_t* __restrict__ in, uint32_t count, const uint32_t* __restrict__ block_sums,
                                                           uint32_t* __restrict__ out, uint32_t* __restrict__ out2);
```

### openzl_amd/csrc/zl_msm_sort.hip

```cpp
#include "zl_msm_sort.h"



__device__ __forceinline__ bool zl_take_one(const uint32_t* s, uint32_t i, uint32_t* __restrict__ ones_list, uint32_t* __restrict__ ones_count) {
    const bool one = s[0] == 1u && (s[1] | s[2] | s[3] | s[4] | s[5] | s[6] | s[7]) == 0u;
    const uint64_t m = __ballot(one);
    if (m == 0) return false;
    const uint32_t lane = threadIdx.x & 63u;
    uint32_t base = 0;
    if (lane == (uint32_t)__ffsll((long long)m) - 1u) base = atomicAdd(ones_count, (uint32_t)__popcll(m));
    base = __shfl(base, __ffsll((long long)m) - 1);
    if (one) ones_list[base + __popcll(m & ((1ull << lane) - 1ull))] = i;
    return one;
}

__device__ __forceinline__ uint32_t zl_take_sign(uint32_t& top_word, int glv) {
    if (!glv) return 0u;
    const uint32_t sg = top_word >> 31;
    top_word &= 0x7FFFFFFFu;
    return sg;
}
__global__ void __launch_bounds__(64) k_msm_zero_words(uint32_t* __restrict__ p, uint32_t n) {
    if (threadIdx.x < n) p[threadIdx.x] = 0u;
}
template <int MODE>
__global__ void __launch_bounds__(256) k_msm_digits(const uint32_t* __restrict__ scalars, uint32_t n, int c, int W,
                                                    uint32_t* __restrict__ counters, uint32_t* __restrict__ entries,
                                                    uint32_t* __restrict__ ones_list, uint32_t* __restrict__ ones_count, const uint8_t* __restrict__ inf,
                                                    int sc_bits, uint32_t* __restrict__ bad) {
    uint32_t i = blockIdx.x * blockDim.x + threadIdx.x;
    const bool live = i < n && !(inf && inf[i]);
    const uint32_t* s = scalars + (size_t)(live ? i : 0) * 8;
    uint32_t sv[8];
    for (int k = 0; k < 8; k++) sv[k] = live ? s[k] : 0u;
    if (MODE == 0) zl_flag_wide_scalar(sv[7], sc_bits, bad);
    if (MODE == 0) {
        if (zl_take_one(sv, i, ones_list, ones_count)) return;
    } else if (sv[0] == 1u && (sv[1] | sv[2] | sv[3] | sv[4] | sv[5] | sv[6] | sv[7]) == 0u) {
        return;
    }
    if (!live) return;
    const uint32_t H = 1u << (c - 1);
    uint32_t carry = 0;
    for (int w = 0; w < W; w++) {
        uint32_t d = zl_get_bits(s, w * c, c) + carry;
        uint32_t neg = 0;
        carry = 0;
        if (d > H) { d = (2 * H) - d; neg = 1; carry = 1; }
        if (d == 0) continue;
        uint32_t bucket = (uint32_t)w * H + (d - 1);
        if (MODE == 0) {
            atomicAdd(&counters[bucket], 1u);
        } else {
            uint32_t pos = atomicAdd(&counters[bucket], 1u);
            entries[pos] = i | (neg << 31);
        }
    }
}

__global__ void __launch_bounds__(256) k_msm_recode(const uint32_t* __restrict__ scalars, uint32_t n, int c, int W, int spread_t, int glv, uint16_t* __restrict__ digits,
                                                             uint32_t* __restrict__ ones_list, uint32_t* __restrict__ ones_count, const uint8_t* __restrict__ inf,
                                                             int sc_bits, uint32_t* __restrict__ bad) {
    ZL_SIDE_PRIO();
    const uint32_t i = blockIdx.x * blockDim.x + threadIdx.x;
    const bool live = i < n;
    const uint4* sp = reinterpret_cast<const uint4*>(scalars + (size_t)(live ? i : 0) * 8);
    uint4 lo = sp[0], hi = sp[1];
    if (live) zl_flag_wide_scalar(hi.w, sc_bits, bad);
    if (!live || (inf && inf[i])) lo = hi = make_uint4(0, 0, 0, 0);
    uint32_t s[8] = {lo.x, lo.y, lo.z, lo.w, hi.x, hi.y, hi.z, hi.w};
    if (zl_take_one(s, i, ones_list, ones_count)) s[0] = 0;
    if (!live) return;
    const uint32_t sg = zl_take_sign(s[7], glv);
    const uint32_t H = 1u << (c - 1);
    uint32_t carry = 0;
    for (int w = 0; w < W; w++) {
        const int pos = w * c;
        const int word = pos >> 5, sh = pos & 31;
        uint64_t v = 0;
#pragma unroll
        for (int k = 0; k < 8; k++) {
            if (k == word) v |= s[k];
            if (k == word + 1) v |= (uint64_t)s[k] << 32;
        }
        uint32_t d = ((uint32_t)(v >> sh) & ((1u << c) - 1)) + carry;
        uint32_t neg = 0;
        carry = 0;
        if (d > H - sg) { d = 2 * H - d; neg = 1; carry = 1; }
        uint32_t b = d - 1;
        if (spread_t >= 0 && w == W - 1) b |= (i & ((1u << (c - 1 - spread_t)) - 1u)) << spread_t;
        digits[(size_t)w * n + i] = d == 0 ? (uint16_t)0xFFFF : (uint16_t)(((neg ^ sg) << 15) | b);
    }
}
__global__ void __launch_bounds__(1024) k_msm_hist_lds(const uint16_t* __restrict__ digits, uint32_t n, uint32_t H, uint32_t per_slice, uint32_t NB,
                                                        uint32_t* __restrict__ counts) {
    ZL_SIDE_PRIO();
    extern __shared__ __attribute__((aligned(16))) unsigned char smem[];
    uint32_t* hist = reinterpret_cast<uint32_t*>(smem);
    const uint32_t slice = blockIdx.x, w = blockIdx.y;
    for (uint32_t b = threadIdx.x; b < H; b += blockDim.x) hist[b] = 0;
    __syncthreads();
    const uint32_t lo = slice * per_slice, hi = min(n, lo + per_slice);
    const uint16_t* dw = digits + (size_t)w * n;
    {
        const size_t row0 = (size_t)w * n;
        uint32_t a = lo, b = hi;
        while (a < b && ((row0 + a) & 7)) a++;
        b = a + ((b - a) & ~7u);
        for (uint32_t i = lo + threadIdx.x; i < a; i += blockDim.x) {
            const uint32_t code = dw[i];
            if (code != 0xFFFFu) atomicAdd(&hist[code & 0x7FFFu], 1u);
        }
        const uint4* dv = reinterpret_cast<const uint4*>(dw + a);
        for (uint32_t j = threadIdx.x; j < (b - a) / 8; j += blockDim.x) {
            const uint4 v = dv[j];
            const uint32_t words[4] = {v.x, v.y, v.z, v.w};
#pragma unroll
            for (int k = 0; k < 8; k++) {
                const uint32_t code = (words[k >> 1] >> ((k & 1) * 16)) & 0xFFFFu;
                if (code != 0xFFFFu) atomicAdd(&hist[code & 0x7FFFu], 1u);
            }
        }
        for (uint32_t i = b + threadIdx.x; i < hi; i += blockDim.x) {
            const uint32_t code = dw[i];
            if (code != 0xFFFFu) atomicAdd(&hist[code & 0x7FFFu], 1u);
        }
    }
    __syncthreads();
    uint32_t* out = counts + (size_t)slice * NB + (size_t)w * H;
    for (uint32_t b = threadIdx.x; b < H; b += blockDim.x) out[b] = hist[b];
}
__global__ void __launch_bounds__(256) k_msm_slice_prefix(uint32_t* __restrict__ counts, uint32_t NB, uint32_t nslices, uint32_t* __restrict__ tot) {
    ZL_SIDE_PRIO();
    const uint32_t b = blockIdx.x * blockDim.x + threadIdx.x;
    if (b >= NB) return;
    uint32_t run = 0;
    for (uint32_t sl = 0; sl < nslices; sl++) {
        const uint32_t v = counts[(size_t)sl * NB + b];
        counts[(size_t)sl * NB + b] = run;
        run += v;
    }
    tot[b] = run;
}
__global__ void __launch_bounds__(1024) k_msm_scatter_range(const uint16_t* __restrict__ digits, uint32_t n, uint32_t H, uint32_t RB,
                                                                     const uint32_t* __restrict__ offsets, uint32_t* __restrict__ entries,
                                                                     const uint32_t* __restrict__ slice_prefix, uint32_t NB, uint32_t nslices, uint32_t per_slice,
                                                                     uint32_t parts, uint32_t W) {
    ZL_SIDE_PRIO();
    extern __shared__ __attribute__((aligned(16))) unsigned char smem[];
    uint32_t* cur = reinterpret_cast<uint32_t*>(smem);
    const uint32_t ranges = gridDim.y, xcd = blockIdx.x & 7u, jj = blockIdx.x >> 3;
    const uint32_t w = xcd + 8u * jj, range = blockIdx.y, part = blockIdx.z;
    if (w >= W) return;
    (void)ranges;
    const uint32_t b0 = range * RB;
    const uint32_t s0 = (uint32_t)((uint64_t)part * nslices / parts), s1 = (uint32_t)((uint64_t)(part + 1) * nslices / parts);
    const uint32_t lo = min(n, s0 * per_slice), hi = part + 1 == parts ? n : min(n, s1 * per_slice);
    const uint32_t* os = offsets + (size_t)w * H + b0;
    const uint32_t* sp = slice_prefix + (size_t)s0 * NB + (size_t)w * H + b0;
    for (uint32_t b = threadIdx.x; b < RB; b += blockDim.x) cur[b] = (b0 + b < H) ? os[b] + (parts > 1 ? sp[b] : 0u) : 0;
    __syncthreads();
    const uint16_t* dw = digits + (size_t)w * n;
    auto take1 = [&](uint32_t i) {
        const uint32_t code = dw[i];
        const uint32_t bucket = code & 0x7FFFu;
        if (code != 0xFFFFu && bucket - b0 < RB) {
            const uint32_t pos = atomicAdd(&cur[bucket - b0], 1u);
            entries[pos] = i | ((code >> 15) << 31);
        }
    };
    auto take8 = [&](const uint4& v, uint32_t i0) {
        uint32_t mask = 0;
#pragma unroll
        for (int k = 0; k < 8; k++) {
            const uint32_t word = k < 2 ? v.x : (k < 4 ? v.y : (k < 6 ? v.z : v.w));
            const uint32_t code = (word >> ((k & 1) * 16)) & 0xFFFFu;
            if (code != 0xFFFFu && (code & 0x7FFFu) - b0 < RB) mask |= 1u << k;
        }
        while (mask) {
            const uint32_t k = (uint32_t)__builtin_ctz(mask);
            mask &= mask - 1u;
            const uint32_t word = k < 2 ? v.x : (k < 4 ? v.y : (k < 6 ? v.z : v.w));
            const uint32_t code = (word >> ((k & 1u) * 16u)) & 0xFFFFu;
            const uint32_t pos = atomicAdd(&cur[(code & 0x7FFFu) - b0], 1u);
            entries[pos] = (i0 + k) | ((code >> 15) << 31);
        }
    };
    const size_t row0 = (size_t)w * n;
    uint32_t a = lo, e = hi;
    while (a < e && ((row0 + a) & 7)) a++;
    e = a + ((e - a) & ~7u);
    for (uint32_t i = lo + threadIdx.x; i < a; i += blockDim.x) take1(i);
    const uint4* dv = reinterpret_cast<const uint4*>(dw + a);
    const uint32_t cnt8 = (e - a) / 8, stride = blockDim.x;
    uint32_t j = threadIdx.x;
    for (; j + stride < cnt8; j += 2 * stride) {
        const uint4 v0 = dv[j], v1 = dv[j + stride];
        take8(v0, a + j * 8);
        take8(v1, a + (j + stride) * 8);
    }
    for (; j < cnt8; j += stride) take8(dv[j], a + j * 8);
    for (uint32_t i = e + threadIdx.x; i < hi; i += blockDim.x) take1(i);
}

__global__ void __launch_bounds__(256) k_msm_recode_wide(const uint32_t* __restrict__ scalars, uint32_t n, int c, int W, uint32_t gw, int spread_t, int glv,
                                                                  uint16_t* __restrict__ lo16, uint8_t* __restrict__ hi8,
                                                                  uint32_t* __restrict__ ones_list, uint32_t* __restrict__ ones_count, const uint8_t* __restrict__ inf,
                                                                  int sc_bits, uint32_t* __restrict__ bad) {
    ZL_SIDE_PRIO();
    const uint32_t i = blockIdx.x * blockDim.x + threadIdx.x;
    const bool live = i < n;
    const uint4* sp = reinterpret_cast<const uint4*>(scalars + (size_t)(live ? i : 0) * 8);
    uint4 lo = sp[0], hi = sp[1];
    if (live) zl_flag_wide_scalar(hi.w, sc_bits, bad);
    if (!live || (inf && inf[i])) lo = hi = make_uint4(0, 0, 0, 0);
    uint32_t s[8] = {lo.x, lo.y, lo.z, lo.w, hi.x, hi.y, hi.z, hi.w};
    if (zl_take_one(s, i, ones_list, ones_count)) s[0] = 0;
    if (!live) return;
    const uint32_t sg = zl_take_sign(s[7], glv);
    const uint32_t H = 1u << (c - 1);
    uint32_t carry = 0;
    for (int w = 0; w < W; w++) {
        const int pos = w * c;
        const int word = pos >> 5, sh = pos & 31;
        uint64_t v = 0;
#pragma unroll
        for (int k = 0; k < 8; k++) {
            if (k == word) v |= s[k];
            if (k == word + 1) v |= (uint64_t)s[k] << 32;
        }
        uint32_t d = ((uint32_t)(v >> sh) & ((1u << c) - 1)) + carry;
        uint32_t neg = 0;
        carry = 0;
        if (d > H) { d = 2 * H - d; neg = 1; carry = 1; }
        uint32_t b = d - 1;
        if (spread_t >= 0 && w == W - 1) b |= (i & ((1u << (c - 1 - spread_t)) - 1u)) << spread_t;
        lo16[(size_t)w * n + i] = (uint16_t)((b & 0x7FFFu) | ((neg ^ sg) << 15));
        hi8[(size_t)w * n + i] = d == 0 ? (uint8_t)0xFF : (uint8_t)((uint32_t)w * gw + (b >> 15));
    }
}
__global__ void __launch_bounds__(256) k_msm_part_hist(const uint8_t* __restrict__ hi8, uint32_t n, uint32_t W, uint32_t G, uint32_t per_slice,
                                                                uint32_t nslices, uint32_t* __restrict__ counts) {
    ZL_SIDE_PRIO();
    __shared__ uint32_t hist[256];
    const uint32_t slice = blockIdx.x, w = blockIdx.y;
    hist[threadIdx.x] = 0;
    __syncthreads();
    const uint32_t lo = slice * per_slice, hi = min(n, lo + per_slice);
    const uint8_t* hw = hi8 + (size_t)w * n;
    const bool al = ((((size_t)w * n) | lo) & 15) == 0;
    const uint32_t body1 = al ? lo + ((hi - lo) & ~15u) : lo;
    const uint4* hv = reinterpret_cast<const uint4*>(hw);
    for (uint32_t i16 = lo / 16 + threadIdx.x; i16 < body1 / 16; i16 += blockDim.x) {
        const uint4 v = hv[i16];
        const uint32_t words[4] = {v.x, v.y, v.z, v.w};
#pragma unroll
        for (int k = 0; k < 16; k++) {
            const uint32_t g = (words[k >> 2] >> ((k & 3) * 8)) & 0xFFu;
            if (g != 0xFFu) atomicAdd(&hist[g], 1u);
        }
    }
    for (uint32_t i = body1 + threadIdx.x; i < hi; i += blockDim.x) {
        const uint32_t g = hw[i];
        if (g != 0xFFu) atomicAdd(&hist[g], 1u);
    }
    __syncthreads();
    if (threadIdx.x < G) counts[((size_t)threadIdx.x * W + w) * nslices + slice] = hist[threadIdx.x];
}
__device__ __forceinline__ void zl_group_range(const uint32_t* __restrict__ part_off, uint32_t g, uint32_t G, uint32_t stride, uint32_t E, uint32_t& s,
                                               uint32_t& e) {
    s = part_off[(size_t)g * stride];
    e = (g + 1 < G) ? part_off[(size_t)(g + 1) * stride] : E;
}
__global__ void __launch_bounds__(256) k_msm_sub_hist(const uint16_t* __restrict__ part_lo, const uint32_t* __restrict__ part_off, uint32_t G,
                                                               uint32_t stride, const uint32_t* __restrict__ total, uint32_t fslices,
                                                               uint32_t* __restrict__ counts) {
    ZL_SIDE_PRIO();
    __shared__ uint32_t hist[128];
    const uint32_t slice = blockIdx.x, g = blockIdx.y;
    if (threadIdx.x < 128) hist[threadIdx.x] = 0;
    __syncthreads();
    uint32_t s, e;
    zl_group_range(part_off, g, G, stride, *total, s, e);
    const uint32_t per = (e - s + fslices - 1) / fslices;
    const uint32_t lo = min(e, s + slice * per), hi = min(e, lo + per);
    const uint32_t body0 = min(hi, (lo + 7u) & ~7u), body1 = max(body0, hi & ~7u);
    for (uint32_t j = lo + threadIdx.x; j < body0; j += blockDim.x) atomicAdd(&hist[(part_lo[j] >> 8) & 127u], 1u);
    const uint4* dv = reinterpret_cast<const uint4*>(part_lo);
    for (uint32_t j8 = body0 / 8 + threadIdx.x; j8 < body1 / 8; j8 += blockDim.x) {
        const uint4 v = dv[j8];
        const uint32_t words[4] = {v.x, v.y, v.z, v.w};
#pragma unroll
        for (int k = 0; k < 8; k++) atomicAdd(&hist[((words[k >> 1] >> ((k & 1) * 16)) >> 8) & 127u], 1u);
    }
    for (uint32_t j = body1 + threadIdx.x; j < hi; j += blockDim.x) atomicAdd(&hist[(part_lo[j] >> 8) & 127u], 1u);
    __syncthreads();
    if (threadIdx.x < 128) counts[((size_t)g * 128 + threadIdx.x) * fslices + slice] = hist[threadIdx.x];
}
struct PartStage {
    uint32_t gcur[256];
    uint32_t hist[256];
    uint32_t start[257];
    uint32_t idx[ZL_PT];
    uint16_t code[ZL_PT];
};
__device__ __forceinline__ void zl_part_scan(PartStage& st) {
    __shared__ uint32_t wsum[4];
    const uint32_t v = st.hist[threadIdx.x];
    uint32_t x = v;
#pragma unroll
    for (int off = 1; off < 64; off <<= 1) {
        const uint32_t y = __shfl_up(x, off);
        if ((threadIdx.x & 63) >= (uint32_t)off) x += y;
    }
    if ((threadIdx.x & 63) == 63) wsum[threadIdx.x >> 6] = x;
    __syncthreads();
    uint32_t base = 0;
    for (uint32_t w = 0; w < (threadIdx.x >> 6); w++) base += wsum[w];
    st.start[threadIdx.x] = base + x - v;
    if (threadIdx.x == 255) st.start[256] = base + x;
    __syncthreads();
}
template <class BinFn, class OutFn>
__device__ __forceinline__ void zl_part_flush(PartStage& st, uint32_t cnt, uint16_t* __restrict__ out_lo, uint32_t* __restrict__ out_idx, BinFn binfn, OutFn outfn) {
    for (uint32_t j = threadIdx.x; j < cnt; j += 256) {
        const uint32_t code = st.code[j];
        const uint32_t b = binfn(code);
        const uint32_t dest = st.gcur[b] + (j - st.start[b]);
        out_lo[dest] = (uint16_t)outfn(code);
        out_idx[dest] = st.idx[j];
    }
    __syncthreads();
    st.gcur[threadIdx.x] += st.hist[threadIdx.x];
    st.hist[threadIdx.x] = 0;
    __syncthreads();
}
__global__ void __launch_bounds__(256) k_msm_part_scatter_st(const uint16_t* __restrict__ lo16, const uint8_t* __restrict__ hi8, uint32_t n, uint32_t W,
                                                                      uint32_t G, uint32_t per_slice, uint32_t nslices, const uint32_t* __restrict__ part_off,
                                                                      uint32_t table_stride, uint32_t first, uint16_t* __restrict__ out_lo,
                                                                      uint32_t* __restrict__ out_idx) {
    ZL_SIDE_PRIO();
    __shared__ PartStage st;
    __shared__ uint8_t grp[ZL_PT];
    const uint32_t slice = blockIdx.x, w = blockIdx.y;
    st.gcur[threadIdx.x] = threadIdx.x < G ? part_off[((size_t)threadIdx.x * W + w) * nslices + slice] : 0u;
    st.hist[threadIdx.x] = 0;
    __syncthreads();
    const uint32_t lo = slice * per_slice, hi = min(n, lo + per_slice);
    const uint8_t* hw = hi8 + (size_t)w * n;
    const uint16_t* lw = lo16 + (size_t)w * n;
    const uint32_t add = w * table_stride + first;
    const bool al = ((((size_t)w * n) | lo) & 15) == 0;
    constexpr int EPT = ZL_PT / 256;
    for (uint32_t t0 = lo; t0 < hi; t0 += ZL_PT) {
        const uint32_t j0 = t0 + threadIdx.x * EPT;
        uint32_t g[EPT], code[EPT], rank[EPT];
        if (al && j0 + EPT <= hi) {
            const uint4 v = *reinterpret_cast<const uint4*>(hw + j0);
            const uint4 l0 = *reinterpret_cast<const uint4*>(lw + j0), l1 = *reinterpret_cast<const uint4*>(lw + j0 + 8);
            const uint32_t words[4] = {v.x, v.y, v.z, v.w};
            const uint32_t lws[8] = {l0.x, l0.y, l0.z, l0.w, l1.x, l1.y, l1.z, l1.w};
#pragma unroll
            for (int k = 0; k < EPT; k++) {
                g[k] = (words[k >> 2] >> ((k & 3) * 8)) & 0xFFu;
                code[k] = (lws[k >> 1] >> ((k & 1) * 16)) & 0xFFFFu;
            }
        } else {
#pragma unroll
            for (int k = 0; k < EPT; k++) {
                const bool ok = j0 + k < hi;
                g[k] = ok ? hw[j0 + k] : 0xFFu;
                code[k] = ok ? lw[j0 + k] : 0u;
            }
        }
#pragma unroll
        for (int k = 0; k < EPT; k++) rank[k] = g[k] != 0xFFu ? atomicAdd(&st.hist[g[k]], 1u) : 0u;
        __syncthreads();
        zl_part_scan(st);
#pragma unroll
        for (int k = 0; k < EPT; k++) {
            if (g[k] != 0xFFu) {
                const uint32_t pos = st.start[g[k]] + rank[k];
                st.code[pos] = (uint16_t)code[k];
                st.idx[pos] = add + j0 + k;
                grp[pos] = (uint8_t)g[k];
            }
        }
        __syncthreads();
        const uint32_t cnt = st.start[256];
        for (uint32_t j = threadIdx.x; j < cnt; j += 256) {
            const uint32_t b = grp[j];
            const uint32_t dest = st.gcur[b] + (j - st.start[b]);
            out_lo[dest] = st.code[j];
            out_idx[dest] = st.idx[j];
        }
        __syncthreads();
        st.gcur[threadIdx.x] += st.hist[threadIdx.x];
        st.hist[threadIdx.x] = 0;
        __syncthreads();
    }
}
__global__ void __launch_bounds__(256) k_msm_sub_scatter_st(const uint16_t* __restrict__ part_lo, const uint32_t* __restrict__ part_idx,
                                                                     const uint32_t* __restrict__ part_off, uint32_t G, uint32_t stride,
                                                                     const uint32_t* __restrict__ total, uint32_t fslices, const uint32_t* __restrict__ sub_off,
                                                                     uint16_t* __restrict__ out_lo, uint32_t* __restrict__ out_idx) {
    ZL_SIDE_PRIO();
    __shared__ PartStage st;
    const uint32_t slice = blockIdx.x, g = blockIdx.y;
    st.gcur[threadIdx.x] = threadIdx.x < 128 ? sub_off[((size_t)g * 128 + threadIdx.x) * fslices + slice] : 0u;
    st.hist[threadIdx.x] = 0;
    __syncthreads();
    uint32_t s, e;
    zl_group_range(part_off, g, G, stride, *total, s, e);
    const uint32_t per = (e - s + fslices - 1) / fslices;
    const uint32_t lo = min(e, s + slice * per), hi = min(e, lo + per);
    constexpr int EPT = ZL_PT / 256;
    const uint32_t a0 = lo & ~7u;
    for (uint32_t t0 = a0; t0 < hi; t0 += ZL_PT) {
        const uint32_t j0 = t0 + threadIdx.x * EPT;
        uint32_t code[EPT], idx[EPT], rank[EPT];
        bool ok[EPT];
        if (j0 >= lo && j0 + EPT <= hi) {
            const uint4 c0 = *reinterpret_cast<const uint4*>(part_lo + j0), c1 = *reinterpret_cast<const uint4*>(part_lo + j0 + 8);
            const uint4* iv = reinterpret_cast<const uint4*>(part_idx + j0);
            const uint4 i0 = iv[0], i1 = iv[1], i2 = iv[2], i3 = iv[3];
            const uint32_t cw[8] = {c0.x, c0.y, c0.z, c0.w, c1.x, c1.y, c1.z, c1.w};
            const uint32_t iw[16] = {i0.x, i0.y, i0.z, i0.w, i1.x, i1.y, i1.z, i1.w, i2.x, i2.y, i2.z, i2.w, i3.x, i3.y, i3.z, i3.w};
#pragma unroll
            for (int k = 0; k < EPT; k++) {
                code[k] = (cw[k >> 1] >> ((k & 1) * 16)) & 0xFFFFu;
                idx[k] = iw[k];
                ok[k] = true;
            }
        } else {
#pragma unroll
            for (int k = 0; k < EPT; k++) {
                ok[k] = j0 + k >= lo && j0 + k < hi;
                code[k] = ok[k] ? part_lo[j0 + k] : 0u;
                idx[k] = ok[k] ? part_idx[j0 + k] : 0u;
            }
        }
#pragma unroll
        for (int k = 0; k < EPT; k++) rank[k] = ok[k] ? atomicAdd(&st.hist[(code[k] >> 8) & 127u], 1u) : 0u;
        __syncthreads();
        zl_part_scan(st);
#pragma unroll
        for (int k = 0; k < EPT; k++) {
            if (ok[k]) {
                const uint32_t pos = st.start[(code[k] >> 8) & 127u] + rank[k];
                st.code[pos] = (uint16_t)code[k];
                st.idx[pos] = idx[k];
            }
        }
        __syncthreads();
        zl_part_flush(st, st.start[256], out_lo, out_idx, [](uint32_t c) { return (c >> 8) & 127u; },
                      [](uint32_t c) { return (c & 0xFFu) | (c & 0x8000u); });
    }
}
__global__ void __launch_bounds__(256) k_msm_fine_hist(const uint16_t* __restrict__ lo2, const uint32_t* __restrict__ sub_off, uint32_t SG,
                                                                uint32_t fslices, const uint32_t* __restrict__ total, uint32_t* __restrict__ counts) {
    ZL_SIDE_PRIO();
    __shared__ uint32_t hist[256];
    const uint32_t sg = blockIdx.x;
    hist[threadIdx.x] = 0;
    __syncthreads();
    const uint32_t s = sub_off[(size_t)sg * fslices], e = (sg + 1 < SG) ? sub_off[(size_t)(sg + 1) * fslices] : *total;
    const uint32_t body0 = min(e, (s + 7u) & ~7u), body1 = max(body0, e & ~7u);
    for (uint32_t j = s + threadIdx.x; j < body0; j += blockDim.x) atomicAdd(&hist[lo2[j] & 0xFFu], 1u);
    const uint4* dv = reinterpret_cast<const uint4*>(lo2);
    for (uint32_t j8 = body0 / 8 + threadIdx.x; j8 < body1 / 8; j8 += blockDim.x) {
        const uint4 v = dv[j8];
        const uint32_t words[4] = {v.x, v.y, v.z, v.w};
#pragma unroll
        for (int k = 0; k < 8; k++) atomicAdd(&hist[(words[k >> 1] >> ((k & 1) * 16)) & 0xFFu], 1u);
    }
    for (uint32_t j = body1 + threadIdx.x; j < e; j += blockDim.x) atomicAdd(&hist[lo2[j] & 0xFFu], 1u);
    __syncthreads();
    counts[(size_t)sg * 256 + threadIdx.x] = hist[threadIdx.x];
}
__global__ void __launch_bounds__(1024) k_msm_fine_sort(const uint16_t* __restrict__ lo2, const uint32_t* __restrict__ idx2,
                                                                const uint32_t* __restrict__ sub_off, uint32_t SG, uint32_t fslices,
                                                                const uint32_t* __restrict__ total, const uint32_t* __restrict__ offsets, uint32_t cap,
                                                                uint32_t* __restrict__ entries, unsigned long long* __restrict__ big_head,
                                                                uint32_t* __restrict__ big_items) {
    ZL_SIDE_PRIO();
    extern __shared__ __attribute__((aligned(16))) unsigned char smem[];
    uint32_t* cur = reinterpret_cast<uint32_t*>(smem);
    uint32_t* stage = cur + 256;
    const uint32_t sg = blockIdx.x;
    const uint32_t s = sub_off[(size_t)sg * fslices], e = (sg + 1 < SG) ? sub_off[(size_t)(sg + 1) * fslices] : *total;
    const uint32_t base = offsets[(size_t)sg * 256];
    const uint32_t len = e - s;
    if (len > cap) {
        if (threadIdx.x == 0) {
            const uint32_t tiles = (len + ZL_BT - 1) / ZL_BT;
            const unsigned long long old = atomicAdd(big_head, (1ull << 32) | tiles);
            const uint32_t item = (uint32_t)(old >> 32);
            big_items[2 * item] = sg;
            big_items[2 * item + 1] = (uint32_t)old;
        }
        return;
    }
    for (uint32_t b = threadIdx.x; b < 256; b += blockDim.x) cur[b] = offsets[(size_t)sg * 256 + b] - base;
    __syncthreads();
    for (uint32_t j = s + threadIdx.x; j < e; j += blockDim.x) {
        const uint32_t code = lo2[j];
        const uint32_t pos = atomicAdd(&cur[code & 0xFFu], 1u);
        stage[pos] = idx2[j] | ((code >> 15) << 31);
    }
    __syncthreads();
    for (uint32_t k = threadIdx.x; k < len; k += blockDim.x) entries[base + k] = stage[k];
}
__global__ void __launch_bounds__(1024) k_msm_fine_sort_big(const uint16_t* __restrict__ lo2, const uint32_t* __restrict__ idx2,
                                                                    const uint32_t* __restrict__ sub_off, uint32_t SG, uint32_t fslices,
                                                                    const uint32_t* __restrict__ total, const unsigned long long* __restrict__ big_head,
                                                                    const uint32_t* __restrict__ big_items, uint32_t* __restrict__ cursor,
                                                                    uint32_t* __restrict__ entries) {
    ZL_SIDE_PRIO();
    __shared__ uint32_t hist[256], start[257], gbase[256], wsum[4], item_sg, item_tile0;
    extern __shared__ __attribute__((aligned(16))) unsigned char smem[];
    uint32_t* stage = reinterpret_cast<uint32_t*>(smem);
    const unsigned long long head = *big_head;
    const uint32_t items = (uint32_t)(head >> 32), tiles = (uint32_t)head;
    constexpr int EPT = ZL_BT / 1024;
    for (uint32_t g = blockIdx.x; g < tiles; g += gridDim.x) {
        if (threadIdx.x == 0) {
            uint32_t lo = 0, hi = items;
            while (hi - lo > 1) {
                const uint32_t mid = (lo + hi) >> 1;
                if (big_items[2 * mid + 1] <= g) lo = mid; else hi = mid;
            }
            item_sg = big_items[2 * lo];
            item_tile0 = big_items[2 * lo + 1];
        }
        if (threadIdx.x < 256) hist[threadIdx.x] = 0;
        __syncthreads();
        const uint32_t sg = item_sg;
        const uint32_t s = sub_off[(size_t)sg * fslices], e = (sg + 1 < SG) ? sub_off[(size_t)(sg + 1) * fslices] : *total;
        const uint32_t t0 = s + (g - item_tile0) * ZL_BT, t1 = min(e, t0 + ZL_BT), cnt = t1 - t0;
        uint32_t val[EPT], bin[EPT], rank[EPT];
#pragma unroll
        for (int k = 0; k < EPT; k++) {
            const uint32_t j = t0 + k * 1024 + threadIdx.x;
            bin[k] = 0xFFFFFFFFu;
            if (j < t1) {
                const uint32_t code = lo2[j];
                val[k] = idx2[j] | ((code >> 15) << 31);
                bin[k] = code & 0xFFu;
                rank[k] = atomicAdd(&hist[bin[k]], 1u);
            }
        }
        __syncthreads();
        if (threadIdx.x < 256) {
            const uint32_t v = hist[threadIdx.x];
            uint32_t x = v;
#pragma unroll
            for (int off = 1; off < 64; off <<= 1) {
                const uint32_t y = __shfl_up(x, off);
                if ((threadIdx.x & 63) >= (uint32_t)off) x += y;
            }
            if ((threadIdx.x & 63) == 63) wsum[threadIdx.x >> 6] = x;
            gbase[threadIdx.x] = v ? atomicAdd(&cursor[(size_t)sg * 256 + threadIdx.x], v) : 0u;
            hist[threadIdx.x] = x - v;
        }
        __syncthreads();
        if (threadIdx.x < 256) {
            uint32_t wb = 0;
            for (uint32_t w = 0; w < (threadIdx.x >> 6); w++) wb += wsum[w];
            start[threadIdx.x] = hist[threadIdx.x] + wb;
            if (threadIdx.x == 255) start[256] = cnt;
        }
        __syncthreads();
#pragma unroll
        for (int k = 0; k < EPT; k++)
            if (bin[k] != 0xFFFFFFFFu) stage[start[bin[k]] + rank[k]] = val[k];
        __syncthreads();
        for (uint32_t j = threadIdx.x; j < cnt; j += 1024) {
            uint32_t lo = 0, hi = 256;
            while (hi - lo > 1) {
                const uint32_t mid = (lo + hi) >> 1;
                if (start[mid] <= j) lo = mid; else hi = mid;
            }
            entries[gbase[lo] + (j - start[lo])] = stage[j];
        }
        __syncthreads();
    }
}

__global__ void __launch_bounds__(SCAN_BLOCK) k_scan_block_sums(const uint32_t* __restrict__ in, uint32_t count, uint32_t* __restrict__ block_sums) {
    ZL_SIDE_PRIO();
    __shared__ uint32_t sh[SCAN_BLOCK];
    uint32_t base = blockIdx.x * SCAN_BLOCK * SCAN_ITEMS + threadIdx.x * SCAN_ITEMS;
    uint32_t s = 0;
    for (int k = 0; k < SCAN_ITEMS; k++) if (base + k < count) s += in[base + k];
    sh[threadIdx.x] = s;
    __syncthreads();
    for (int off = SCAN_BLOCK / 2; off > 0; off >>= 1) {
        if (threadIdx.x < off) sh[threadIdx.x] += sh[threadIdx.x + off];
        __syncthreads();
    }
    if (threadIdx.x == 0) block_sums[blockIdx.x] = sh[0];
}
__global__ void __launch_bounds__(1024) k_scan_top(uint32_t* __restrict__ block_sums, uint32_t nblocks, uint32_t* __restrict__ total_out,
                                                          const uint32_t* __restrict__ flag_in ) {
    ZL_SIDE_PRIO();
    __shared__ uint32_t sh[1024];
    __shared__ uint32_t carry;
    if (threadIdx.x == 0) carry = 0;
    __syncthreads();
    for (uint32_t base = 0; base < nblocks; base += 1024) {
        uint32_t idx = base + threadIdx.x;
        uint32_t v = idx < nblocks ? block_sums[idx] : 0;
        sh[threadIdx.x] = v;
        __syncthreads();
        for (int off = 1; off < 1024; off <<= 1) {
            uint32_t t = threadIdx.x >= off ? sh[threadIdx.x - off] : 0;
            __syncthreads();
            sh[threadIdx.x] += t;
            __syncthreads();
        }
        uint32_t incl = sh[threadIdx.x];
        if (idx < nblocks) block_sums[idx] = carry + incl - v;
        __syncthreads();
        if (threadIdx.x == 1023) carry += incl;
        __syncthreads();
    }
    if (threadIdx.x == 0) {
        *total_out = carry;
        if (flag_in) total_out[1] = *flag_in;
    }
}
__global__ void __launch_bounds__(1024) k_msm_prefix_small(uint32_t* __restrict__ counts, uint32_t NB, uint32_t nslices, uint32_t* __restrict__ offsets,
                                                                  uint32_t* __restrict__ cursor, const uint32_t* __restrict__ flag_in) {
    ZL_SIDE_PRIO();
    extern __shared__ __attribute__((aligned(16))) unsigned char smem[];
    uint32_t* tot = reinterpret_cast<uint32_t*>(smem);
    __shared__ uint32_t sh[1024];
    for (uint32_t b = threadIdx.x; b < NB; b += 1024) {
        uint32_t run = 0;
        for (uint32_t sl = 0; sl < nslices; sl++) {
            const uint32_t x = counts[(size_t)sl * NB + b];
            counts[(size_t)sl * NB + b] = run;
            run += x;
        }
        tot[b + (b >> 4)] = run;
    }
    __syncthreads();
    const uint32_t base = threadIdx.x * 16;
    uint32_t s = 0;
#pragma unroll
    for (int k = 0; k < 16; k++)
        if (base + k < NB) s += tot[threadIdx.x * 17 + k];
    sh[threadIdx.x] = s;
    __syncthreads();
    for (int off = 1; off < 1024; off <<= 1) {
        const uint32_t t = threadIdx.x >= (uint32_t)off ? sh[threadIdx.x - off] : 0;
        __syncthreads();
        sh[threadIdx.x] += t;
        __syncthreads();
    }
    uint32_t run = sh[threadIdx.x] - s;
#pragma unroll
    for (int k = 0; k < 16; k++)
        if (base + k < NB) {
            const uint32_t x = tot[threadIdx.x * 17 + k];
            tot[threadIdx.x * 17 + k] = run;
            run += x;
        }
    __syncthreads();
    for (uint32_t b = threadIdx.x; b < NB; b += 1024) {
        const uint32_t o = tot[b + (b >> 4)];
        offsets[b] = o;
        cursor[b] = o;
    }
    if (threadIdx.x == 1023) {
        offsets[NB] = sh[1023];
        if (flag_in) offsets[NB + 1] = *flag_in;
    }
}
__global__ void __launch_bounds__(SCAN_BLOCK) k_scan_apply(const uint32_t* __restrict__ in, uint32_t count, const uint32_t* __restrict__ block_sums,
                                                           uint32_t* __restrict__ out, uint32_t* __restrict__ out2) {
    ZL_SIDE_PRIO();
    __shared__ uint32_t sh[SCAN_BLOCK];
    uint32_t base = blockIdx.x * SCAN_BLOCK * SCAN_ITEMS + threadIdx.x * SCAN_ITEMS;
    uint32_t v[SCAN_ITEMS];
    uint32_t s = 0;
    for (int k = 0; k < SCAN_ITEMS; k++) { v[k] = (base + k < count) ? in[base + k] : 0; s += v[k]; }
    sh[threadIdx.x] = s;
    __syncthreads();
    for (int off = 1; off < SCAN_BLOCK; off <<= 1) {
        uint32_t t = threadIdx.x >= off ? sh[threadIdx.x - off] : 0;
        __syncthreads();
        sh[threadIdx.x] += t;
        __syncthreads();
    }
    uint32_t run = block_sums[blockIdx.x] + sh[threadIdx.x] - s;
    for (int k = 0; k < SCAN_ITEMS; k++) {
        if (base + k < count) { out[base + k] = run; out2[base + k] = run; }
        run += v[k];
    }
}

template __global__ void k_msm_digits<0>(const uint32_t*, uint32_t, int, int, uint32_t*, uint32_t*, uint32_t*, uint32_t*, const uint8_t*, int, uint32_t*);
template __global__ void k_msm_digits<1>(const uint32_t*, uint32_t, int, int, uint32_t*, uint32_t*, uint32_t*, uint32_t*, const uint8_t*, int, uint32_t*);
```

Before: 488.8 million points/s.

## Fuse wide recode with partition histogram and pass chunk heads to merge

Merges the per-window partition histogram into the wide recode kernel: each block walks a span of scalars with software prefetch, counts group hits in LDS, and adds them atomically into zeroed global counts. This removes the separate pass that re-read the hi8 array. The accumulate kernel now records each chunk's first bucket so merge_cuts can skip its own search. The change also adjusts the merge_cuts occupancy bound and the reduce-tree grid sizing. In exchange it adds a memset, global atomics and LDS pressure in the recode kernel.

```diff
diff --git a/openzl_amd/csrc/zl_msm_accumulate.h b/openzl_amd/csrc/zl_msm_accumulate.h
--- a/openzl_amd/csrc/zl_msm_accumulate.h
+++ b/openzl_amd/csrc/zl_msm_accumulate.h
@@ -25,13 +25,15 @@
                                                     const Affine<typename HotField<typename G::F>::type>* __restrict__ bases,
                                                     XYZZ<typename HotField<typename G::F>::type>* __restrict__ bucket_sums,
                                                     XYZZ<typename HotField<typename G::F>::type>* __restrict__ partials, uint32_t ZL_CHUNK,
-                                                    const Affine<typename HotField<typename G::F>::type>* __restrict__ phib, uint32_t n_real, uint32_t idx_mask = 0x7fffffffu) {
+                                                    const Affine<typename HotField<typename G::F>::type>* __restrict__ phib, uint32_t n_real, uint32_t* __restrict__ chunk_head,
+                                                    uint32_t idx_mask = 0x7fffffffu) {
     using F = typename HotField<typename G::F>::type;
     const uint64_t start64 = (uint64_t)t * ZL_CHUNK;
     if (start64 >= E) return;
     const uint32_t start = (uint32_t)start64;
     const uint32_t end = (uint32_t)min((uint64_t)E, start64 + ZL_CHUNK);
     uint32_t b = zl_upper_bound(offsets, NB + 1, start) - 1;
+    if (!QUAD || sub == 0) chunk_head[t] = b;
     uint32_t b_start = offsets[b], b_end = offsets[b + 1];
     XYZZ<F> acc = XYZZ<F>::inf();
     for (uint32_t e = start; e < end; e++) {
@@ -65,12 +67,12 @@
                                                         const Affine<typename G::F>* __restrict__ bases_,
                                                         XYZZ<typename G::F>* __restrict__ bucket_sums_,
                                                         XYZZ<typename G::F>* __restrict__ partials_, uint32_t ZL_CHUNK,
-                                                        const Affine<typename G::F>* __restrict__ phib_, uint32_t n_real) {
+                                                        const Affine<typename G::F>* __restrict__ phib_, uint32_t n_real, uint32_t* __restrict__ chunk_head) {
     using F = typename HotField<typename G::F>::type;
     static_assert(sizeof(F) == sizeof(typename G::F), "hot flavour must share the layout");
     zl_accumulate_chunk<G>(blockIdx.x * blockDim.x + threadIdx.x, 0, offsets[NB], entries, offsets, NB, reinterpret_cast<const Affine<F>*>(bases_),
                            reinterpret_cast<XYZZ<F>*>(bucket_sums_), reinterpret_cast<XYZZ<F>*>(partials_), ZL_CHUNK,
-                           reinterpret_cast<const Affine<F>*>(phib_) - n_real, n_real);
+                           reinterpret_cast<const Affine<F>*>(phib_) - n_real, n_real, chunk_head);
 }
 #ifdef ZL_MEASURE
 template <class G>
@@ -78,13 +80,13 @@
                                                         const Affine<typename G::F>* __restrict__ bases_,
                                                         XYZZ<typename G::F>* __restrict__ bucket_sums_,
                                                         XYZZ<typename G::F>* __restrict__ partials_, uint32_t ZL_CHUNK,
-                                                        const Affine<typename G::F>* __restrict__ phib_, uint32_t n_real, unsigned long long* __restrict__ clk, uint32_t idx_mask) {
+                                                        const Affine<typename G::F>* __restrict__ phib_, uint32_t n_real, uint32_t* __restrict__ chunk_head, unsigned long long* __restrict__ clk, uint32_t idx_mask) {
     if constexpr (G::COORDS == 1) {
         using F = typename HotField<typename G::F>::type;
         const unsigned long long c0 = __builtin_readcyclecounter(), w0 = __builtin_amdgcn_s_memrealtime();
         zl_accumulate_chunk<G>(blockIdx.x * blockDim.x + threadIdx.x, 0, offsets[NB], entries, offsets, NB, reinterpret_cast<const Affine<F>*>(bases_),
                                reinterpret_cast<XYZZ<F>*>(bucket_sums_), reinterpret_cast<XYZZ<F>*>(partials_), ZL_CHUNK,
-                               reinterpret_cast<const Affine<F>*>(phib_) - n_real, n_real, idx_mask);
+                               reinterpret_cast<const Affine<F>*>(phib_) - n_real, n_real, chunk_head, idx_mask);
         const unsigned long long c1 = __builtin_readcyclecounter(), w1 = __builtin_amdgcn_s_memrealtime();
         if (threadIdx.x == 0) {
             unsigned long long* o = clk + (size_t)4 * blockIdx.x;
@@ -98,12 +100,12 @@
                                                         const Affine<typename G::F>* __restrict__ bases_,
                                                         XYZZ<typename G::F>* __restrict__ bucket_sums_,
                                                         XYZZ<typename G::F>* __restrict__ partials_, uint32_t ZL_CHUNK,
-                                                        const Affine<typename G::F>* __restrict__ phib_, uint32_t n_real) {
+                                                        const Affine<typename G::F>* __restrict__ phib_, uint32_t n_real, uint32_t* __restrict__ chunk_head) {
     using F = typename HotField<typename G::F>::type;
     const uint32_t gt = blockIdx.x * blockDim.x + threadIdx.x;
     zl_accumulate_chunk<G, true>(gt >> 2, (int)(gt & 3u), offsets[NB], entries, offsets, NB, reinterpret_cast<const Affine<F>*>(bases_),
                                  reinterpret_cast<XYZZ<F>*>(bucket_sums_), reinterpret_cast<XYZZ<F>*>(partials_), ZL_CHUNK,
-                                 reinterpret_cast<const Affine<F>*>(phib_) - n_real, n_real);
+                                 reinterpret_cast<const Affine<F>*>(phib_) - n_real, n_real, chunk_head);
 }
 #ifndef ZL_ACC_PAIR_WAVES
 #define ZL_ACC_PAIR_WAVES 2
@@ -152,14 +154,14 @@
     else pair_store(&partials[(size_t)2 * t + (b_start <= start ? 0 : 1)], half, acc);
 }
 #ifdef ZL_MEASURE
-#define ZL_MSM_ACCUMULATE_CLK_KERNEL(X, G) X template __global__ void k_msm_accumulate_clk<G>(const uint32_t*, const uint32_t*, uint32_t, const Affine<typename G::F>*, XYZZ<typename G::F>*, XYZZ<typename G::F>*, uint32_t, const Affine<typename G::F>*, uint32_t, unsigned long long*, uint32_t);
+#define ZL_MSM_ACCUMULATE_CLK_KERNEL(X, G) X template __global__ void k_msm_accumulate_clk<G>(const uint32_t*, const uint32_t*, uint32_t, const Affine<typename G::F>*, XYZZ<typename G::F>*, XYZZ<typename G::F>*, uint32_t, const Affine<typename G::F>*, uint32_t, uint32_t*, unsigned long long*, uint32_t);
 #else
 #define ZL_MSM_ACCUMULATE_CLK_KERNEL(X, G)
 #endif
 #define ZL_MSM_ACCUMULATE_KERNELS_G1(X, G) \
     ZL_MSM_ACCUMULATE_CLK_KERNEL(X, G) \
-    X template __global__ void k_msm_accumulate<G>(const uint32_t*, const uint32_t*, uint32_t, const Affine<typename G::F>*, XYZZ<typename G::F>*, XYZZ<typename G::F>*, uint32_t, const Affine<typename G::F>*, uint32_t); \
-    X template __global__ void k_msm_accumulate_quad<G>(const uint32_t*, const uint32_t*, uint32_t, const Affine<typename G::F>*, XYZZ<typename G::F>*, XYZZ<typename G::F>*, uint32_t, const Affine<typename G::F>*, uint32_t);
+    X template __global__ void k_msm_accumulate<G>(const uint32_t*, const uint32_t*, uint32_t, const Affine<typename G::F>*, XYZZ<typename G::F>*, XYZZ<typename G::F>*, uint32_t, const Affine<typename G::F>*, uint32_t, uint32_t*); \
+    X template __global__ void k_msm_accumulate_quad<G>(const uint32_t*, const uint32_t*, uint32_t, const Affine<typename G::F>*, XYZZ<typename G::F>*, XYZZ<typename G::F>*, uint32_t, const Affine<typename G::F>*, uint32_t, uint32_t*);
 #define ZL_MSM_ACCUMULATE_KERNELS_G2(X, G) \
     X template __global__ void k_msm_accumulate_pair<G, true>(const uint32_t*, const uint32_t*, uint32_t, const Affine<typename G::F>*, XYZZ<typename G::F>*, XYZZ<typename G::F>*, uint32_t, const Affine<typename G::F>*, uint32_t); \
     X template __global__ void k_msm_accumulate_pair<G, false>(const uint32_t*, const uint32_t*, uint32_t, const Affine<typename G::F>*, XYZZ<typename G::F>*, XYZZ<typename G::F>*, uint32_t, const Affine<typename G::F>*, uint32_t);
diff --git a/openzl_amd/csrc/zl_msm_job.h b/openzl_amd/csrc/zl_msm_job.h
--- a/openzl_amd/csrc/zl_msm_job.h
+++ b/openzl_amd/csrc/zl_msm_job.h
@@ -95,7 +95,7 @@
     const zl_bases* bsp = nullptr;
     uint32_t *d_counts = nullptr, *d_offsets = nullptr, *d_cursor = nullptr, *d_entries = nullptr, *d_block_sums = nullptr, *d_big_list = nullptr,
              *d_big_count = nullptr, *d_ones_count = nullptr, *d_giant_count = nullptr, *d_giant_list = nullptr, *d_ones_list = nullptr,
-             *d_bigsg_items = nullptr, *d_bad_scalar = nullptr;
+             *d_bigsg_items = nullptr, *d_bad_scalar = nullptr, *d_chunk_head = nullptr;
     unsigned long long* d_bigsg_head = nullptr;
     X *d_buckets = nullptr, *d_partials = nullptr, *d_segs = nullptr, *d_stage1 = nullptr, *d_sets = nullptr, *d_ones_parts = nullptr, *d_giant_tmp = nullptr;
     const Affine<F>* d_bases = nullptr;
@@ -249,7 +249,7 @@
             d_sort_b = (unsigned char*)p;
         }
         const size_t max_bigsg = (size_t)(maxE / 1024) + 2;
-        size_t small_words = (size_t)3 * (NB + 1) + 1 + scan_blocks + 1 + max_big + max_giant + 16 + n + 2 * max_bigsg;
+        size_t small_words = (size_t)3 * (NB + 1) + 1 + scan_blocks + 1 + max_big + max_giant + 16 + n + 2 * max_bigsg + nchunks;
         if ((rc = zl_scratch_get(ctx, slots.data[0], small_words * 4, &p))) return rc;
         d_counts = (uint32_t*)p;
         d_offsets = d_counts + (NB + 1);
@@ -263,6 +263,7 @@
         d_giant_list = d_big_count + 16;
         d_ones_list = d_giant_list + max_giant;
         d_bigsg_items = d_ones_list + n;
+        d_chunk_head = d_bigsg_items + 2 * max_bigsg;
         d_bigsg_head = reinterpret_cast<unsigned long long*>((reinterpret_cast<uintptr_t>(d_big_count + 4) + 7) & ~(uintptr_t)7);
         if ((rc = zl_scratch_get(ctx, slots.data[1], maxE * 4, &p))) return rc;
         d_entries = (uint32_t*)p;
@@ -341,13 +342,13 @@
         const int glv_i = glv ? 1 : 0;
         (void)hipFuncSetAttribute(reinterpret_cast<const void*>(&k_msm_hist_lds), hipFuncAttributeMaxDynamicSharedMemorySize, 128 * 1024);
         (void)hipFuncSetAttribute(reinterpret_cast<const void*>(&k_msm_scatter_range), hipFuncAttributeMaxDynamicSharedMemorySize, 128 * 1024);
-        if (wide) sort_wide(st, sc_eff, inf_eff, bad_eff, nblk, glv_i);
+        if (wide) sort_wide(st, sc_eff, inf_eff, bad_eff, glv_i);
         else if (c <= 16) sort_lds(st, sc_eff, inf_eff, bad_eff, nblk, glv_i);
         else sort_atomics(st, nblk);
         ZL_HIP(ctx, hipGetLastError());
         return ZL_OK;
     }
-    void sort_wide(hipStream_t st, const uint32_t* sc_eff, const uint8_t* inf_eff, uint32_t* bad_eff, uint32_t nblk, int glv_i) {
+    void sort_wide(hipStream_t st, const uint32_t* sc_eff, const uint8_t* inf_eff, uint32_t* bad_eff, int glv_i) {
         const zl_bases& bs = *bsp;
         const uint32_t nslices = lay.nslices, per_slice = lay.per_slice, P = lay.P, pscan_blocks = lay.pscan_blocks;
         uint16_t* d_lo16 = (uint16_t*)d_sort_a;
@@ -357,8 +358,10 @@
         uint32_t* d_pcounts = (uint32_t*)(d_sort_a + lay.pcounts);
         uint32_t* d_poff = d_pcounts + P;
         uint32_t* d_pblock = d_poff + P + 1;
-        hipLaunchKernelGGL(k_msm_recode_wide, dim3(nblk), dim3(256), 0, st, sc_eff, (uint32_t)n, c, W, pre ? 0u : (H >> 15), spread_t, glv_i, d_lo16, d_hi8, d_ones_list, d_ones_count, inf_eff, sc_bits, bad_eff);
-        hipLaunchKernelGGL(k_msm_part_hist, dim3(nslices, W), dim3(256), 0, st, d_hi8, (uint32_t)n, (uint32_t)W, Gn, per_slice, nslices, d_pcounts);
+        const uint32_t span = 256u * std::min<uint32_t>(32u, std::max<uint32_t>(1u, (uint32_t)(n >> 19)));
+        (void)hipMemsetAsync(d_pcounts, 0, (size_t)P * 4, st);
+        hipLaunchKernelGGL(k_msm_recode_wide, dim3((per_slice + span - 1) / span, nslices), dim3(256), zl_recode_wide_lds(Gn, (uint32_t)W, pre ? 0u : (H >> 15)), st, sc_eff, (uint32_t)n, c, W, pre ? 0u : (H >> 15), spread_t, glv_i,
+                           d_lo16, d_hi8, d_ones_list, d_ones_count, inf_eff, sc_bits, bad_eff, Gn, per_slice, span, nslices, d_pcounts);
         hipLaunchKernelGGL(k_scan_block_sums, dim3(pscan_blocks), dim3(SCAN_BLOCK), 0, st, d_pcounts, P, d_pblock);
         hipLaunchKernelGGL(k_scan_top, dim3(1), dim3(1024), 0, st, d_pblock, pscan_blocks, d_poff + P, (const uint32_t*)nullptr);
         hipLaunchKernelGGL(k_scan_apply, dim3(pscan_blocks), dim3(SCAN_BLOCK), 0, st, d_pcounts, P, d_pblock, d_poff, d_pcounts);
@@ -434,18 +437,18 @@
         } else {
             if (quad)
                 hipLaunchKernelGGL((k_msm_accumulate_quad<G>), dim3((4 * nchunks + ZL_ACC_BLOCK - 1) / ZL_ACC_BLOCK), dim3(ZL_ACC_BLOCK), 0, st, d_entries, d_offsets, NB, d_bases, d_buckets, d_partials, ZL_CHUNK,
-                                   glv ? d_phi : d_bases, glv ? (uint32_t)n_real : 0xFFFFFFFFu);
+                                   glv ? d_phi : d_bases, glv ? (uint32_t)n_real : 0xFFFFFFFFu, d_chunk_head);
 #ifdef ZL_MEASURE
             else if (ctx->acc_clk && (size_t)((nchunks + ZL_ACC_BLOCK - 1) / ZL_ACC_BLOCK) * 32 <= ctx->acc_clk_cap) {
                 ctx->acc_clk_waves = (nchunks + ZL_ACC_BLOCK - 1) / ZL_ACC_BLOCK;
                 hipLaunchKernelGGL((k_msm_accumulate_clk<G>), dim3((nchunks + ZL_ACC_BLOCK - 1) / ZL_ACC_BLOCK), dim3(ZL_ACC_BLOCK), 0, st, d_entries, d_offsets, NB, d_bases, d_buckets, d_partials, ZL_CHUNK,
-                                   glv ? d_phi : d_bases, glv ? (uint32_t)n_real : 0xFFFFFFFFu, (unsigned long long*)ctx->acc_clk,
+                                   glv ? d_phi : d_bases, glv ? (uint32_t)n_real : 0xFFFFFFFFu, d_chunk_head, (unsigned long long*)ctx->acc_clk,
                                    zl_tune("ZL_TUNE_ACC_CLK_IDX_BITS", 31) >= 31 ? 0x7fffffffu : ((1u << zl_tune("ZL_TUNE_ACC_CLK_IDX_BITS", 31)) - 1u));
             }
 #endif
             else
                 hipLaunchKernelGGL((k_msm_accumulate<G>), dim3((nchunks + ZL_ACC_BLOCK - 1) / ZL_ACC_BLOCK), dim3(ZL_ACC_BLOCK), 0, st, d_entries, d_offsets, NB, d_bases, d_buckets, d_partials, ZL_CHUNK,
-                                   glv ? d_phi : d_bases, glv ? (uint32_t)n_real : 0xFFFFFFFFu);
+                                   glv ? d_phi : d_bases, glv ? (uint32_t)n_real : 0xFFFFFFFFu, d_chunk_head);
         }
         ZL_HIP(ctx, hipGetLastError());
         return ZL_OK;
@@ -463,7 +466,7 @@
                 hipLaunchKernelGGL((k_msm_merge_pair<G, true>), dim3((NB + 7) / 8), dim3(64), 0, st, d_offsets, NB, d_buckets, d_partials, d_big_list, d_big_count, d_giant_list, d_giant_count, ZL_CHUNK, big_span);
         } else {
             if (by_cuts)
-                hipLaunchKernelGGL((k_msm_merge_cuts<G>), dim3((nchunks + 63) / 64), dim3(64), 0, st, d_offsets, NB, d_buckets, d_partials, d_big_list, d_big_count, d_giant_list, d_giant_count, ZL_CHUNK, big_span, nchunks);
+                hipLaunchKernelGGL((k_msm_merge_cuts<G>), dim3((nchunks + 63) / 64), dim3(64), 0, st, d_offsets, d_chunk_head, NB, d_buckets, d_partials, d_big_list, d_big_count, d_giant_list, d_giant_count, ZL_CHUNK, big_span, nchunks);
             else if (NB > quad_max)
                 hipLaunchKernelGGL((k_msm_merge<G>), dim3((NB + 63) / 64), dim3(64), 0, st, d_offsets, NB, d_buckets, d_partials, d_big_list, d_big_count, d_giant_list, d_giant_count, ZL_CHUNK, big_span);
             else
@@ -510,8 +513,11 @@
                     else
                         hipLaunchKernelGGL((k_msm_reduce_tree_pair<G, true>), dim3((lanes + 7) / 8), dim3(64), 0, st, cur, nxt, lv, nodes, lanes);
                 } else {
-                    if (lanes > quad_max)
-                        hipLaunchKernelGGL((k_msm_reduce_tree<G>), dim3((lanes + 63) / 64), dim3(64), 0, st, cur, nxt, lv, nodes, lanes);
+                    if (lanes > quad_max) {
+                        uint32_t add_blocks, copy_blocks;
+                        zl_tree_blocks<G>(lv, SETS * nodes, add_blocks, copy_blocks);
+                        hipLaunchKernelGGL((k_msm_reduce_tree<G>), dim3(add_blocks + copy_blocks), dim3(64), 0, st, cur, nxt, lv, nodes, lanes);
+                    }
                     else
                         hipLaunchKernelGGL((k_msm_reduce_tree<G, true>), dim3((4 * lanes + 63) / 64), dim3(64), 0, st, cur, nxt, lv, nodes, lanes);
                 }
diff --git a/openzl_amd/csrc/zl_msm_reduce.h b/openzl_amd/csrc/zl_msm_reduce.h
--- a/openzl_amd/csrc/zl_msm_reduce.h
+++ b/openzl_amd/csrc/zl_msm_reduce.h
@@ -46,7 +46,8 @@
     bucket_sums[b] = XYZZ<typename G::F>::inf();
 }
 template <class G>
-__global__ void __launch_bounds__(64, sizeof(XYZZ<typename G::F>) <= 256 ? 3 : 1) k_msm_merge_cuts(const uint32_t* __restrict__ offsets, uint32_t NB, XYZZ<typename G::F>* __restrict__ bucket_sums,
+__global__ void __launch_bounds__(64, sizeof(XYZZ<typename G::F>) <= 256 ? 2 : 1) k_msm_merge_cuts(const uint32_t* __restrict__ offsets, const uint32_t* __restrict__ chunk_head, uint32_t NB,
+                                                   XYZZ<typename G::F>* __restrict__ bucket_sums,
                                                    const XYZZ<typename G::F>* __restrict__ partials, uint32_t* __restrict__ big_list,
                                                    uint32_t* __restrict__ big_count, uint32_t* __restrict__ giant_list, uint32_t* __restrict__ giant_count,
                                                    uint32_t ZL_CHUNK, uint32_t big_span, uint32_t nchunks) {
@@ -57,15 +58,15 @@
     const uint64_t p64 = (uint64_t)t * ZL_CHUNK;
     if (p64 >= offsets[NB]) return;
     const uint32_t p = (uint32_t)p64;
-    const uint32_t b = zl_bucket_of_entry(offsets, NB, p);
+    const uint32_t b = chunk_head[t];
     const uint32_t s = offsets[b], e = offsets[b + 1];
     if (s == p || s / ZL_CHUNK != t - 1) return;
     const uint32_t t0 = t - 1, t1 = (e - 1) / ZL_CHUNK;
     if (t1 - t0 + 1 > ZL_GIANT_SPAN) { giant_list[atomicAdd(giant_count, 1u)] = b; return; }
     if (t1 - t0 + 1 > big_span) { big_list[atomicAdd(big_count, 1u)] = b; return; }
-    XYZZ<F> acc = XYZZ<F>::inf();
-    for (uint32_t tt = t0; tt <= t1; tt++) {
-        const XYZZ<F> q = partials[(size_t)2 * tt + (s <= tt * ZL_CHUNK ? 0 : 1)];
+    XYZZ<F> acc = partials[(size_t)2 * t0 + (s == t0 * ZL_CHUNK ? 0 : 1)];
+    for (uint32_t tt = t; tt <= t1; tt++) {
+        const XYZZ<F> q = partials[(size_t)2 * tt];
         zl::add_full(acc, q);
     }
     bucket_sums[b] = acc;
@@ -239,27 +240,56 @@
     if (flat) out[(size_t)2 * t + 1] = run;
     else out[(size_t)2 * t + 1] = wsum;
 }
+template <class G>
+struct TreeCopy { static constexpr uint32_t VECS = sizeof(XYZZ<typename G::F>) / 16; };
+template <class G>
+inline void zl_tree_blocks(uint32_t level, uint32_t total_nodes, uint32_t& add_blocks, uint32_t& copy_blocks) {
+    add_blocks = (uint32_t)(((uint64_t)total_nodes * (level + 1) + 63) / 64);
+    copy_blocks = (uint32_t)(((uint64_t)total_nodes * TreeCopy<G>::VECS + 63) / 64);
+}
 template <class G, bool QUAD = false>
 __global__ void __launch_bounds__(64) k_msm_reduce_tree(const XYZZ<typename G::F>* __restrict__ in, XYZZ<typename G::F>* __restrict__ out, uint32_t level,
                                                          uint32_t nodes_out_per_set, uint32_t total_lanes) {
     ZL_SIDE_PRIO();
     using X = XYZZ<typename G::F>;
-    const uint32_t gt = blockIdx.x * blockDim.x + threadIdx.x;
-    const uint32_t t = QUAD ? gt >> 2 : gt;
-    const int sub = QUAD ? (int)(gt & 3u) : 0;
-    if (t >= total_lanes) return;
     const uint32_t ch_out = level + 2, ch_in = level + 1;
-    const uint32_t ch = t % ch_out, node = (t / ch_out) % nodes_out_per_set, set = t / (ch_out * nodes_out_per_set);
-    const size_t left = ((size_t)set * nodes_out_per_set * 2 + (size_t)2 * node) * ch_in, right = left + ch_in;
-    if (ch == ch_out - 1) {
-        if (sub == 0) out[t] = in[right];
-        return;
-    }
-    X acc = in[left + ch];
-    const X o = in[right + ch];
-    if constexpr (QUAD) zl::add_full_quad(acc, o, sub);
-    else zl::add_full(acc, o);
-    if (sub == 0) out[t] = acc;
+    if constexpr (!QUAD) {
+        static_assert(sizeof(X) % 16 == 0 && alignof(X) <= 16, "the top channel is copied in 16-byte vectors");
+        const uint32_t total_nodes = total_lanes / ch_out;
+        const uint32_t add_lanes = total_nodes * ch_in, add_blocks = (add_lanes + 63) / 64;
+        if (blockIdx.x >= add_blocks) {
+            const uint32_t j = (blockIdx.x - add_blocks) * 64 + threadIdx.x;
+            const uint32_t g = j / TreeCopy<G>::VECS, v = j % TreeCopy<G>::VECS;
+            if (g >= total_nodes) return;
+            const uint4* src = reinterpret_cast<const uint4*>(in + ((size_t)2 * g + 1) * ch_in);
+            uint4* dst = reinterpret_cast<uint4*>(out + (size_t)g * ch_out + ch_in);
+            dst[v] = src[v];
+            return;
+        }
+        const uint32_t t = blockIdx.x * 64 + threadIdx.x;
+        if (t >= add_lanes) return;
+        const uint32_t g = t / ch_in, ch = t % ch_in;
+        const size_t left = (size_t)2 * g * ch_in, right = left + ch_in;
+        X acc = in[left + ch];
+        const X o = in[right + ch];
+        zl::add_full(acc, o);
+        out[(size_t)g * ch_out + ch] = acc;
+    } else {
+        const uint32_t gt = blockIdx.x * blockDim.x + threadIdx.x;
+        const uint32_t t = gt >> 2;
+        const int sub = (int)(gt & 3u);
+        if (t >= total_lanes) return;
+        const uint32_t ch = t % ch_out, node = (t / ch_out) % nodes_out_per_set, set = t / (ch_out * nodes_out_per_set);
+        const size_t left = ((size_t)set * nodes_out_per_set * 2 + (size_t)2 * node) * ch_in, right = left + ch_in;
+        if (ch == ch_out - 1) {
+            if (sub == 0) out[t] = in[right];
+            return;
+        }
+        X acc = in[left + ch];
+        const X o = in[right + ch];
+        zl::add_full_quad(acc, o, sub);
+        if (sub == 0) out[t] = acc;
+    }
 }
 template <class G, bool QUAD = false>
 __global__ void __launch_bounds__(64, 2) k_msm_merge_pair(const uint32_t* __restrict__ offsets, uint32_t NB, XYZZ<typename G::F>* __restrict__ bucket_sums,
@@ -471,7 +501,7 @@
     ZL_MSM_TAIL_KERNELS_COMMON(X, G) \
     X template __global__ void k_msm_merge<G, false>(const uint32_t*, uint32_t, XYZZ<typename G::F>*, const XYZZ<typename G::F>*, uint32_t*, uint32_t*, uint32_t*, uint32_t*, uint32_t, uint32_t); \
     X template __global__ void k_msm_merge<G, true>(const uint32_t*, uint32_t, XYZZ<typename G::F>*, const XYZZ<typename G::F>*, uint32_t*, uint32_t*, uint32_t*, uint32_t*, uint32_t, uint32_t); \
-    X template __global__ void k_msm_merge_cuts<G>(const uint32_t*, uint32_t, XYZZ<typename G::F>*, const XYZZ<typename G::F>*, uint32_t*, uint32_t*, uint32_t*, uint32_t*, uint32_t, uint32_t, uint32_t); \
+    X template __global__ void k_msm_merge_cuts<G>(const uint32_t*, const uint32_t*, uint32_t, XYZZ<typename G::F>*, const XYZZ<typename G::F>*, uint32_t*, uint32_t*, uint32_t*, uint32_t*, uint32_t, uint32_t, uint32_t); \
     X template __global__ void k_msm_merge_big<G>(const uint32_t*, XYZZ<typename G::F>*, const XYZZ<typename G::F>*, const uint32_t*, const uint32_t*, uint32_t); \
     X template __global__ void k_msm_merge_giant<G>(const uint32_t*, XYZZ<typename G::F>*, const XYZZ<typename G::F>*, const uint32_t*, const uint32_t*, uint32_t); \
     X template __global__ void k_msm_merge_giant2<G>(XYZZ<typename G::F>*, const XYZZ<typename G::F>*, const uint32_t*, const uint32_t*); \
diff --git a/openzl_amd/csrc/zl_msm_sort.h b/openzl_amd/csrc/zl_msm_sort.h
--- a/openzl_amd/csrc/zl_msm_sort.h
+++ b/openzl_amd/csrc/zl_msm_sort.h
@@ -25,9 +25,9 @@
 __global__ void __launch_bounds__(256) k_msm_recode_wide(const uint32_t* __restrict__ scalars, uint32_t n, int c, int W, uint32_t gw, int spread_t, int glv,
                                                                   uint16_t* __restrict__ lo16, uint8_t* __restrict__ hi8,
                                                                   uint32_t* __restrict__ ones_list, uint32_t* __restrict__ ones_count, const uint8_t* __restrict__ inf,
-                                                                  int sc_bits, uint32_t* __restrict__ bad);
-__global__ void __launch_bounds__(256) k_msm_part_hist(const uint8_t* __restrict__ hi8, uint32_t n, uint32_t W, uint32_t G, uint32_t per_slice,
-                                                                uint32_t nslices, uint32_t* __restrict__ counts);
+                                                                  int sc_bits, uint32_t* __restrict__ bad, uint32_t G, uint32_t per_slice, uint32_t span, uint32_t nslices,
+                                                                  uint32_t* __restrict__ counts);
+inline size_t zl_recode_wide_lds(uint32_t G, uint32_t W, uint32_t gw) { return (size_t)(gw ? G : G * W) * 4; }
 __global__ void __launch_bounds__(256) k_msm_sub_hist(const uint16_t* __restrict__ part_lo, const uint32_t* __restrict__ part_off, uint32_t G,
                                                                uint32_t stride, const uint32_t* __restrict__ total, uint32_t fslices,
                                                                uint32_t* __restrict__ counts);
diff --git a/openzl_amd/csrc/zl_msm_sort.hip b/openzl_amd/csrc/zl_msm_sort.hip
--- a/openzl_amd/csrc/zl_msm_sort.hip
+++ b/openzl_amd/csrc/zl_msm_sort.hip
@@ -206,66 +206,64 @@
 __global__ void __launch_bounds__(256) k_msm_recode_wide(const uint32_t* __restrict__ scalars, uint32_t n, int c, int W, uint32_t gw, int spread_t, int glv,
                                                                   uint16_t* __restrict__ lo16, uint8_t* __restrict__ hi8,
                                                                   uint32_t* __restrict__ ones_list, uint32_t* __restrict__ ones_count, const uint8_t* __restrict__ inf,
-                                                                  int sc_bits, uint32_t* __restrict__ bad) {
-    ZL_SIDE_PRIO();
-    const uint32_t i = blockIdx.x * blockDim.x + threadIdx.x;
-    const bool live = i < n;
-    const uint4* sp = reinterpret_cast<const uint4*>(scalars + (size_t)(live ? i : 0) * 8);
-    uint4 lo = sp[0], hi = sp[1];
-    if (live) zl_flag_wide_scalar(hi.w, sc_bits, bad);
-    if (!live || (inf && inf[i])) lo = hi = make_uint4(0, 0, 0, 0);
-    uint32_t s[8] = {lo.x, lo.y, lo.z, lo.w, hi.x, hi.y, hi.z, hi.w};
-    if (zl_take_one(s, i, ones_list, ones_count)) s[0] = 0;
-    if (!live) return;
-    const uint32_t sg = zl_take_sign(s[7], glv);
+                                                                  int sc_bits, uint32_t* __restrict__ bad, uint32_t G, uint32_t per_slice, uint32_t span, uint32_t nslices,
+                                                                  uint32_t* __restrict__ counts) {
+    ZL_SIDE_PRIO();
+    extern __shared__ __attribute__((aligned(16))) unsigned char smem[];
+    uint32_t* hist = reinterpret_cast<uint32_t*>(smem);
+    const uint32_t slice = blockIdx.y, cells = gw ? G : G * (uint32_t)W;
+    for (uint32_t k = threadIdx.x; k < cells; k += blockDim.x) hist[k] = 0;
+    __syncthreads();
+    const uint32_t s_hi = min(n, (slice + 1) * per_slice);
+    const uint32_t b0 = min(s_hi, slice * per_slice + blockIdx.x * span), b1 = min(s_hi, b0 + span);
     const uint32_t H = 1u << (c - 1);
-    uint32_t carry = 0;
-    for (int w = 0; w < W; w++) {
-        const int pos = w * c;
-        const int word = pos >> 5, sh = pos & 31;
-        uint64_t v = 0;
-#pragma unroll
-        for (int k = 0; k < 8; k++) {
-            if (k == word) v |= s[k];
-            if (k == word + 1) v |= (uint64_t)s[k] << 32;
-        }
-        uint32_t d = ((uint32_t)(v >> sh) & ((1u << c) - 1)) + carry;
-        uint32_t neg = 0;
-        carry = 0;
-        if (d > H) { d = 2 * H - d; neg = 1; carry = 1; }
-        uint32_t b = d - 1;
-        if (spread_t >= 0 && w == W - 1) b |= (i & ((1u << (c - 1 - spread_t)) - 1u)) << spread_t;
-        lo16[(size_t)w * n + i] = (uint16_t)((b & 0x7FFFu) | ((neg ^ sg) << 15));
-        hi8[(size_t)w * n + i] = d == 0 ? (uint8_t)0xFF : (uint8_t)((uint32_t)w * gw + (b >> 15));
-    }
-}
-__global__ void __launch_bounds__(256) k_msm_part_hist(const uint8_t* __restrict__ hi8, uint32_t n, uint32_t W, uint32_t G, uint32_t per_slice,
-                                                                uint32_t nslices, uint32_t* __restrict__ counts) {
-    ZL_SIDE_PRIO();
-    __shared__ uint32_t hist[256];
-    const uint32_t slice = blockIdx.x, w = blockIdx.y;
-    hist[threadIdx.x] = 0;
-    __syncthreads();
-    const uint32_t lo = slice * per_slice, hi = min(n, lo + per_slice);
-    const uint8_t* hw = hi8 + (size_t)w * n;
-    const bool al = ((((size_t)w * n) | lo) & 15) == 0;
-    const uint32_t body1 = al ? lo + ((hi - lo) & ~15u) : lo;
-    const uint4* hv = reinterpret_cast<const uint4*>(hw);
-    for (uint32_t i16 = lo / 16 + threadIdx.x; i16 < body1 / 16; i16 += blockDim.x) {
-        const uint4 v = hv[i16];
-        const uint32_t words[4] = {v.x, v.y, v.z, v.w};
-#pragma unroll
-        for (int k = 0; k < 16; k++) {
-            const uint32_t g = (words[k >> 2] >> ((k & 3) * 8)) & 0xFFu;
-            if (g != 0xFFu) atomicAdd(&hist[g], 1u);
-        }
-    }
-    for (uint32_t i = body1 + threadIdx.x; i < hi; i += blockDim.x) {
-        const uint32_t g = hw[i];
-        if (g != 0xFFu) atomicAdd(&hist[g], 1u);
-    }
-    __syncthreads();
-    if (threadIdx.x < G) counts[((size_t)threadIdx.x * W + w) * nslices + slice] = hist[threadIdx.x];
+    uint4 nlo = make_uint4(0, 0, 0, 0), nhi = nlo;
+    if (b0 + threadIdx.x < b1) {
+        const uint4* sp = reinterpret_cast<const uint4*>(scalars + (size_t)(b0 + threadIdx.x) * 8);
+        nlo = sp[0]; nhi = sp[1];
+    }
+    for (uint32_t base = b0; base < b1; base += blockDim.x) {
+        const uint32_t i = base + threadIdx.x;
+        const bool live = i < b1;
+        uint4 lo = nlo, hi = nhi;
+        if (i + blockDim.x < b1) {
+            const uint4* sp = reinterpret_cast<const uint4*>(scalars + (size_t)(i + blockDim.x) * 8);
+            nlo = sp[0]; nhi = sp[1];
+        }
+        if (live) zl_flag_wide_scalar(hi.w, sc_bits, bad);
+        if (!live || (inf && inf[i])) lo = hi = make_uint4(0, 0, 0, 0);
+        uint32_t s[8] = {lo.x, lo.y, lo.z, lo.w, hi.x, hi.y, hi.z, hi.w};
+        if (zl_take_one(s, i, ones_list, ones_count)) s[0] = 0;
+        if (!live) continue;
+        const uint32_t sg = zl_take_sign(s[7], glv);
+        uint32_t carry = 0;
+        for (int w = 0; w < W; w++) {
+            const int pos = w * c;
+            const int word = pos >> 5, sh = pos & 31;
+            uint64_t v = 0;
+#pragma unroll
+            for (int k = 0; k < 8; k++) {
+                if (k == word) v |= s[k];
+                if (k == word + 1) v |= (uint64_t)s[k] << 32;
+            }
+            uint32_t d = ((uint32_t)(v >> sh) & ((1u << c) - 1)) + carry;
+            uint32_t neg = 0;
+            carry = 0;
+            if (d > H) { d = 2 * H - d; neg = 1; carry = 1; }
+            uint32_t b = d - 1;
+            if (spread_t >= 0 && w == W - 1) b |= (i & ((1u << (c - 1 - spread_t)) - 1u)) << spread_t;
+            const uint32_t g = (uint32_t)w * gw + (b >> 15);
+            lo16[(size_t)w * n + i] = (uint16_t)((b & 0x7FFFu) | ((neg ^ sg) << 15));
+            hi8[(size_t)w * n + i] = d == 0 ? (uint8_t)0xFF : (uint8_t)g;
+            if (d != 0 && g < G) atomicAdd(&hist[gw ? g : g * (uint32_t)W + (uint32_t)w], 1u);
+        }
+    }
+    __syncthreads();
+    for (uint32_t k = threadIdx.x; k < cells; k += blockDim.x) {
+        const uint32_t v = hist[k];
+        const uint32_t cell = gw ? k * (uint32_t)W + k / gw : k;
+        if (v) atomicAdd(&counts[(size_t)cell * nslices + slice], v);
+    }
 }
 __device__ __forceinline__ void zl_group_range(const uint32_t* __restrict__ part_off, uint32_t g, uint32_t G, uint32_t stride, uint32_t E, uint32_t& s,
                                                uint32_t& e) {
```

Result: faster. 495.4 million points/s, median of 6 (+1.3%).
